# python-graphblas/python-graphblas

Hardware: AMD Instinct MI355X
Metric: GTEPS (mxv) on R-MAT scale-24 (higher is better)
Workload: dtype f32

## Files before the change

include/grb_mi355x.h:

```cpp
#ifndef GRB_MI355X_H
#define GRB_MI355X_H

#include <stdbool.h>
#include <stddef.h>
#include <stdint.h>

#ifdef __cplusplus
extern "C" {
#endif

#define GRB_VERSION 2
#define GRB_SUBVERSION 0

typedef uint64_t GrB_Index;
#define GrB_INDEX_MAX ((GrB_Index)(1ULL << 60) - 1)

typedef enum {
    GrB_SUCCESS = 0,
    GrB_NO_VALUE = 1,
    GrB_UNINITIALIZED_OBJECT = -1,
    GrB_NULL_POINTER = -2,
    GrB_INVALID_VALUE = -3,
    GrB_INVALID_INDEX = -4,
    GrB_DOMAIN_MISMATCH = -5,
// ... 133 lines not shown
    extern GrB_BinaryOp GrB_FIRST_##T, GrB_SECOND_##T, GrB_ONEB_##T, GxB_PAIR_##T, GrB_PLUS_##T, GrB_MINUS_##T,        \
        GrB_TIMES_##T, GrB_MIN_##T, GrB_MAX_##T, GxB_ANY_##T, GxB_LOR_##T, GxB_LAND_##T, GxB_LXOR_##T;                 \
      \
    extern GrB_BinaryOp GrB_EQ_##T, GrB_NE_##T, GrB_GT_##T, GrB_LT_##T, GrB_GE_##T, GrB_LE_##T;                        \
    extern GrB_Monoid GxB_ANY_##T##_MONOID;                                                                            \
    extern GrB_Semiring GxB_ANY_PAIR_##T, GxB_ANY_FIRST_##T, GxB_ANY_SECOND_##T;
GRB_FOR_EACH_TNAME(GRB_DECL_BINOPS)
#undef GRB_DECL_BINOPS
extern GrB_BinaryOp GrB_LOR, GrB_LAND, GrB_LXOR, GrB_LXNOR;
extern GrB_Monoid GrB_LOR_MONOID_BOOL, GrB_LAND_MONOID_BOOL, GrB_LXOR_MONOID_BOOL, GrB_LXNOR_MONOID_BOOL;

#define GRB_DECL_NUMERIC_OPS(T)                                                                                        \
    extern GrB_Monoid GrB_PLUS_MONOID_##T, GrB_TIMES_MONOID_##T, GrB_MIN_MONOID_##T, GrB_MAX_MONOID_##T;               \
    extern GrB_Semiring GrB_PLUS_TIMES_SEMIRING_##T, GrB_PLUS_MIN_SEMIRING_##T, GrB_MIN_PLUS_SEMIRING_##T,             \
        GrB_MIN_TIMES_SEMIRING_##T, GrB_MIN_FIRST_SEMIRING_##T, GrB_MIN_SECOND_SEMIRING_##T,                           \
        GrB_MIN_MAX_SEMIRING_##T, GrB_MAX_PLUS_SEMIRING_##T, GrB_MAX_TIMES_SEMIRING_##T,                               \
        GrB_MAX_FIRST_SEMIRING_##T, GrB_MAX_SECOND_SEMIRING_##T, GrB_MAX_MIN_SEMIRING_##T;                             \
    extern GrB_Semiring GxB_PLUS_PLUS_##T, GxB_PLUS_PAIR_##T, GxB_PLUS_FIRST_##T, GxB_PLUS_SECOND_##T,                 \
        GxB_PLUS_MAX_##T, GxB_MIN_MIN_##T, GxB_MAX_MAX_##T, GxB_MIN_PAIR_##T, GxB_MAX_PAIR_##T, GxB_TIMES_TIMES_##T,   \
        GxB_TIMES_PLUS_##T;
GRB_FOR_EACH_NUMERIC(GRB_DECL_NUMERIC_OPS)
#undef GRB_DECL_NUMERIC_OPS

extern GrB_Semiring GrB_LOR_LAND_SEMIRING_BOOL, GrB_LAND_LOR_SEMIRING_BOOL, GrB_LXOR_LAND_SEMIRING_BOOL,
    GrB_LXNOR_LOR_SEMIRING_BOOL;
extern GrB_Semiring GxB_LOR_LOR_BOOL, GxB_LAND_LAND_BOOL, GxB_LOR_FIRST_BOOL, GxB_LOR_SECOND_BOOL, GxB_LOR_PAIR_BOOL,
    GxB_LAND_FIRST_BOOL, GxB_LAND_SECOND_BOOL, GxB_LOR_LXOR_BOOL, GxB_LAND_LXOR_BOOL, GxB_LXOR_LOR_BOOL,
    GxB_LXOR_LXOR_BOOL, GxB_LXOR_FIRST_BOOL, GxB_LXOR_SECOND_BOOL, GxB_LXOR_PAIR_BOOL;

#define GRB_FOR_EACH_POSITIONAL(X) X(FIRSTI) X(FIRSTI1) X(FIRSTJ) X(FIRSTJ1) X(SECONDI) X(SECONDI1) X(SECONDJ) X(SECONDJ1)
#define GRB_DECL_POSITIONAL(P)                                                                                         \
    extern GrB_BinaryOp GxB_##P##_INT32, GxB_##P##_INT64;                                                              \
    extern GrB_Semiring GxB_MIN_##P##_INT32, GxB_MIN_##P##_INT64, GxB_MAX_##P##_INT32, GxB_MAX_##P##_INT64,            \
        GxB_ANY_##P##_INT32, GxB_ANY_##P##_INT64, GxB_PLUS_##P##_INT32, GxB_PLUS_##P##_INT64;
GRB_FOR_EACH_POSITIONAL(GRB_DECL_POSITIONAL)
#undef GRB_DECL_POSITIONAL


GrB_Info GrX_Matrix_import_CSR_device(GrB_Matrix *A, GrB_Type type, GrB_Index nrows, GrB_Index ncols,
                                      const int64_t *d_Ap, const int32_t *d_Aj, const void *d_Ax, GrB_Index nvals,
                                      int iso, int copy);
GrB_Info GxB_init(GrB_Mode mode, void *(*user_malloc)(size_t), void *(*user_calloc)(size_t, size_t),
                  void *(*user_realloc)(void *, size_t), void (*user_free)(void *));
GrB_Info GxB_Matrix_import_CSR(GrB_Matrix *A, GrB_Type type, GrB_Index nrows, GrB_Index ncols, GrB_Index **Ap, GrB_Index **Aj,
                               void **Ax, GrB_Index Ap_size, GrB_Index Aj_size, GrB_Index Ax_size, bool iso, bool jumbled,
                               const GrB_Descriptor desc);
GrB_Info GxB_Matrix_pack_CSR(GrB_Matrix A, GrB_Index **Ap, GrB_Index **Aj, void **Ax, GrB_Index Ap_size, GrB_Index Aj_size,
                             GrB_Index Ax_size, bool iso, bool jumbled, const GrB_Descriptor desc);
GrB_Info GrX_Matrix_hint_ranked(GrB_Matrix A, int ranked);
GrB_Info GrX_Matrix_shard_setup(GrB_Matrix A, const uint32_t *col_counts, int on_device, const GrB_Matrix like);
GrB_Info GrX_Matrix_export_CSR_device(const int64_t **d_Ap, const int32_t **d_Aj, const void **d_Ax, GrB_Index *nvals,
                                      int *iso, const GrB_Matrix A);
GrB_Info GrX_Vector_import_dense_device(GrB_Vector *v, GrB_Type type, GrB_Index n, const void *d_val,
                                        const uint32_t *d_present);
GrB_Info GrX_Vector_export_dense_device(const void **d_val, const uint32_t **d_present, const GrB_Vector v);
GrB_Info GrX_Vector_pin_natural(GrB_Vector v, int pinned);
GrB_Info GrX_Vector_modified(GrB_Vector v);
GrB_Info GrX_Matrix_cache_transpose(GrB_Matrix A);
GrB_Info GrX_get_stream(void **hip_stream);
GrB_Info GrX_set_stream(void *hip_stream);
GrB_Info GrX_synchronize(void);
GrB_Info GrX_trim_memory(void);
GrB_Info GrX_timer_start(void);
GrB_Info GrX_timer_stop(float *elapsed_ms);
typedef struct {
    int64_t kernel_launches;
    int64_t tiles;
    int64_t flops;
    int64_t out_nvals;
    int32_t method;
    int32_t fused_epilogue;
    int64_t hot_k;
    int64_t long_entries;
    int64_t long_segments;
    int32_t long_kernel;
    int32_t reorders;
    int64_t ordered;
    int64_t value_dict;
    int64_t fill_absent;
    int64_t long_probe;
    int64_t long_tails;
    int64_t pinned_natural;
    int64_t cold_tile_mode;
} GrX_Stats;
GrB_Info GrX_last_stats(GrX_Stats *stats);
GrB_Info GrX_mxm_streamed(const GrB_Semiring semiring, const GrB_Matrix A, const GrB_Matrix B, uint64_t budget_bytes,
                          uint64_t *nvals, uint64_t *checksum, uint64_t *flops, uint64_t *batches);
GrB_Info GrX_Matrix_isclose(bool *result, const GrB_Matrix A, const GrB_Matrix B, double rel_tol, double abs_tol);
GrB_Info GrX_Matrix_dup_as(GrB_Matrix *C, const GrB_Type type, const GrB_Matrix A);
GrB_Info GrX_Vector_dup_as(GrB_Vector *w, const GrB_Type type, const GrB_Vector u);
GrB_Info GrX_Vector_fill_absent(GrB_Vector v, const GrB_Monoid monoid);
GrB_Info GrX_Matrix_cache_bytes(const GrB_Matrix A, uint64_t *bytes);
GrB_Info GrX_option_set(const char *name, int64_t value);
GrB_Info GrX_option_get(const char *name, int64_t *value);
GrB_Info GrX_options_reset(void);
const char *GrX_version_string(void);

#define GRB_DECL_UNARY(T)                                                                                              \
    extern GrB_UnaryOp GrB_IDENTITY_##T, GrB_AINV_##T, GrB_MINV_##T, GrB_ABS_##T, GxB_ONE_##T, GxB_LNOT_##T;           \
    extern GrB_IndexUnaryOp GrB_VALUEEQ_##T, GrB_VALUENE_##T, GrB_VALUEGT_##T, GrB_VALUEGE_##T, GrB_VALUELT_##T,       \
        GrB_VALUELE_##T;                                                                                               \
    extern GrB_BinaryOp GrB_DIV_##T, GxB_RDIV_##T, GxB_RMINUS_##T, GxB_ISEQ_##T, GxB_ISNE_##T, GxB_ISGT_##T,           \
        GxB_ISLT_##T, GxB_ISGE_##T, GxB_ISLE_##T, GxB_POW_##T;
GRB_FOR_EACH_TNAME(GRB_DECL_UNARY)
#undef GRB_DECL_UNARY
extern GrB_UnaryOp GrB_LNOT, GrB_BNOT_INT8, GrB_BNOT_INT16, GrB_BNOT_INT32, GrB_BNOT_INT64, GrB_BNOT_UINT8, GrB_BNOT_UINT16,
    GrB_BNOT_UINT32, GrB_BNOT_UINT64;
extern GrB_IndexUnaryOp GrB_ROWINDEX_INT32, GrB_ROWINDEX_INT64, GrB_COLINDEX_INT32, GrB_COLINDEX_INT64, GrB_DIAGINDEX_INT32,
    GrB_DIAGINDEX_INT64, GrB_TRIL, GrB_TRIU, GrB_DIAG, GrB_OFFDIAG, GrB_COLLE, GrB_COLGT, GrB_ROWLE, GrB_ROWGT;

GrB_Info GrB_Scalar_new(GrB_Scalar *s, GrB_Type type);
GrB_Info GrB_Scalar_dup(GrB_Scalar *s, const GrB_Scalar t);
GrB_Info GrB_Scalar_free(GrB_Scalar *s);
GrB_Info GrB_Scalar_clear(GrB_Scalar s);
GrB_Info GrB_Scalar_nvals(GrB_Index *nvals, const GrB_Scalar s);
GrB_Info GrB_Scalar_wait(GrB_Scalar s, GrB_WaitMode mode);
GrB_Info GrB_Scalar_error(const char **error, const GrB_Scalar s);

GrB_Info GrB_Vector_apply(GrB_Vector w, const GrB_Vector mask, const GrB_BinaryOp accum, const GrB_UnaryOp op, const GrB_Vector u, const GrB_Descriptor desc);
GrB_Info GrB_Matrix_apply(GrB_Matrix C, const GrB_Matrix Mask, const GrB_BinaryOp accum, const GrB_UnaryOp op, const GrB_Matrix A, const GrB_Descriptor desc);
GrB_Info GrB_Vector_eWiseAdd_Semiring(GrB_Vector w, const GrB_Vector mask, const GrB_BinaryOp accum, const GrB_Semiring op, const GrB_Vector u, const GrB_Vector v, const GrB_Descriptor desc);
GrB_Info GrB_Vector_eWiseMult_Semiring(GrB_Vector w, const GrB_Vector mask, const GrB_BinaryOp accum, const GrB_Semiring op, const GrB_Vector u, const GrB_Vector v, const GrB_Descriptor desc);
#define GRB_DECL_MAT_BINARY(FN, HANDLE) \
    GrB_Info FN(GrB_Matrix C, const GrB_Matrix Mask, const GrB_BinaryOp accum, const HANDLE op, const GrB_Matrix A, const GrB_Matrix B, const GrB_Descriptor desc);
GRB_DECL_MAT_BINARY(GrB_Matrix_eWiseAdd_BinaryOp, GrB_BinaryOp)
GRB_DECL_MAT_BINARY(GrB_Matrix_eWiseAdd_Monoid, GrB_Monoid)
GRB_DECL_MAT_BINARY(GrB_Matrix_eWiseAdd_Semiring, GrB_Semiring)
GRB_DECL_MAT_BINARY(GrB_Matrix_eWiseMult_BinaryOp, GrB_BinaryOp)
GRB_DECL_MAT_BINARY(GrB_Matrix_eWiseMult_Monoid, GrB_Monoid)
GRB_DECL_MAT_BINARY(GrB_Matrix_eWiseMult_Semiring, GrB_Semiring)
GrB_Info GxB_Matrix_eWiseUnion(GrB_Matrix C, const GrB_Matrix Mask, const GrB_BinaryOp accum, const GrB_BinaryOp add, const GrB_Matrix A, const GrB_Scalar alpha, const GrB_Matrix B, const GrB_Scalar beta, const GrB_Descriptor desc);
GrB_Info GxB_Vector_eWiseUnion(GrB_Vector w, const GrB_Vector mask, const GrB_BinaryOp accum, const GrB_BinaryOp add, const GrB_Vector u, const GrB_Scalar alpha, const GrB_Vector v, const GrB_Scalar beta, const GrB_Descriptor desc);
GRB_DECL_MAT_BINARY(GrB_Matrix_kronecker_BinaryOp, GrB_BinaryOp)
GRB_DECL_MAT_BINARY(GrB_Matrix_kronecker_Monoid, GrB_Monoid)
GRB_DECL_MAT_BINARY(GrB_Matrix_kronecker_Semiring, GrB_Semiring)
#undef GRB_DECL_MAT_BINARY
GrB_Info GrB_Matrix_assign(GrB_Matrix C, const GrB_Matrix Mask, const GrB_BinaryOp accum, const GrB_Matrix A, const GrB_Index *I, GrB_Index ni, const GrB_Index *J, GrB_Index nj, const GrB_Descriptor desc);
GrB_Info GrB_Row_assign(GrB_Matrix C, const GrB_Vector mask, const GrB_BinaryOp accum, const GrB_Vector u, GrB_Index i, const GrB_Index *J, GrB_Index nj, const GrB_Descriptor desc);
GrB_Info GrB_Col_assign(GrB_Matrix C, const GrB_Vector mask, const GrB_BinaryOp accum, const GrB_Vector u, const GrB_Index *I, GrB_Index ni, GrB_Index j, const GrB_Descriptor desc);
GrB_Info GrB_Matrix_extract(GrB_Matrix C, const GrB_Matrix Mask, const GrB_BinaryOp accum, const GrB_Matrix A, const GrB_Index *I, GrB_Index ni, const GrB_Index *J, GrB_Index nj, const GrB_Descriptor desc);
GrB_Info GrB_Col_extract(GrB_Vector w, const GrB_Vector mask, const GrB_BinaryOp accum, const GrB_Matrix A, const GrB_Index *I, GrB_Index ni, GrB_Index j, const GrB_Descriptor desc);
GrB_Info GrB_Matrix_reduce_BinaryOp(GrB_Vector w, const GrB_Vector mask, const GrB_BinaryOp accum, const GrB_BinaryOp op, const GrB_Matrix A, const GrB_Descriptor desc);
GrB_Info GrB_Matrix_reduce_Monoid_Scalar(GrB_Scalar s, const GrB_BinaryOp accum, const GrB_Monoid monoid, const GrB_Matrix A, const GrB_Descriptor desc);
GrB_Info GrB_Vector_reduce_Monoid_Scalar(GrB_Scalar s, const GrB_BinaryOp accum, const GrB_Monoid monoid, const GrB_Vector u, const GrB_Descriptor desc);
GrB_Info GrB_Matrix_removeElement(GrB_Matrix C, GrB_Index i, GrB_Index j);
GrB_Info GrB_Matrix_diag(GrB_Matrix *C, const GrB_Vector v, int64_t k);
GrB_Info GxB_Vector_diag(GrB_Vector v, const GrB_Matrix A, int64_t k, const GrB_Descriptor desc);
GrB_Info GxB_Matrix_sort(GrB_Matrix C, GrB_Matrix P, GrB_BinaryOp op, const GrB_Matrix A, const GrB_Descriptor desc);
GrB_Info GxB_Vector_sort(GrB_Vector w, GrB_Vector p, GrB_BinaryOp op, const GrB_Vector u, const GrB_Descriptor desc);
GrB_Info GrX_sort_limits(int64_t *wave_max, int64_t *lds_max);
GrB_Info GrX_sort_last(int64_t rows_by_path[3]);
GrB_Info GrX_Matrix_reverse_rows(GrB_Matrix C, const GrB_Matrix A);
GrB_Info GrX_Vector_reverse(GrB_Vector w, const GrB_Vector u);
GrB_Info GrB_Vector_assign_Scalar(GrB_Vector w, const GrB_Vector mask, const GrB_BinaryOp accum, const GrB_Scalar s, const GrB_Index *I, GrB_Index ni, const GrB_Descriptor desc);
GrB_Info GrB_Vector_setElement_Scalar(GrB_Vector w, const GrB_Scalar s, GrB_Index i);
GrB_Info GrB_Vector_extractElement_Scalar(GrB_Scalar s, const GrB_Vector u, GrB_Index i);
GrB_Info GrB_Matrix_assign_Scalar(GrB_Matrix C, const GrB_Matrix Mask, const GrB_BinaryOp accum, const GrB_Scalar s, const GrB_Index *I, GrB_Index ni, const GrB_Index *J, GrB_Index nj, const GrB_Descriptor desc);
GrB_Info GrB_Matrix_setElement_Scalar(GrB_Matrix C, const GrB_Scalar s, GrB_Index i, GrB_Index j);
GrB_Info GrB_Matrix_extractElement_Scalar(GrB_Scalar s, const GrB_Matrix A, GrB_Index i, GrB_Index j);
GrB_Info GrB_Vector_select_Scalar(GrB_Vector w, const GrB_Vector mask, const GrB_BinaryOp accum, const GrB_IndexUnaryOp op, const GrB_Vector u, const GrB_Scalar y, const GrB_Descriptor desc);
GrB_Info GrB_Matrix_select_Scalar(GrB_Matrix C, const GrB_Matrix Mask, const GrB_BinaryOp accum, const GrB_IndexUnaryOp op, const GrB_Matrix A, const GrB_Scalar y, const GrB_Descriptor desc);
GrB_Info GrB_Vector_apply_BinaryOp1st_Scalar(GrB_Vector w, const GrB_Vector mask, const GrB_BinaryOp accum, const GrB_BinaryOp op, const GrB_Scalar x, const GrB_Vector u, const GrB_Descriptor desc);
GrB_Info GrB_Vector_apply_BinaryOp2nd_Scalar(GrB_Vector w, const GrB_Vector mask, const GrB_BinaryOp accum, const GrB_BinaryOp op, const GrB_Vector u, const GrB_Scalar y, const GrB_Descriptor desc);
GrB_Info GrB_Vector_apply_IndexOp_Scalar(GrB_Vector w, const GrB_Vector mask, const GrB_BinaryOp accum, const GrB_IndexUnaryOp op, const GrB_Vector u, const GrB_Scalar y, const GrB_Descriptor desc);
GrB_Info GrB_Matrix_apply_BinaryOp1st_Scalar(GrB_Matrix C, const GrB_Matrix Mask, const GrB_BinaryOp accum, const GrB_BinaryOp op, const GrB_Scalar x, const GrB_Matrix A, const GrB_Descriptor desc);
GrB_Info GrB_Matrix_apply_BinaryOp2nd_Scalar(GrB_Matrix C, const GrB_Matrix Mask, const GrB_BinaryOp accum, const GrB_BinaryOp op, const GrB_Matrix A, const GrB_Scalar y, const GrB_Descriptor desc);
// ... 30 lines not shown
```

python-graphblas_amd/_lib.py:

```python
from __future__ import annotations

import ctypes
import os

_HERE = os.path.dirname(os.path.abspath(__file__))
DEFAULT_LIB = os.path.join(_HERE, "csrc", "libgrb_mi355x.so")

lib = None
_handles = {}

c_void_p = ctypes.c_void_p
c_u64 = ctypes.c_uint64
c_int = ctypes.c_int

TYPE_NAMES = ["BOOL", "INT8", "INT16", "INT32", "INT64", "UINT8", "UINT16", "UINT32", "UINT64", "FP32", "FP64"]

GrB_SUCCESS = 0
GrB_NO_VALUE = 1


class GrX_Stats(ctypes.Structure):
    _fields_ = [("kernel_launches", ctypes.c_int64), ("tiles", ctypes.c_int64), ("flops", ctypes.c_int64),
                ("out_nvals", ctypes.c_int64), ("method", ctypes.c_int32), ("fused_epilogue", ctypes.c_int32),
                ("hot_k", ctypes.c_int64), ("long_entries", ctypes.c_int64), ("long_segments", ctypes.c_int64),
                ("long_kernel", ctypes.c_int32), ("reorders", ctypes.c_int32), ("ordered", ctypes.c_int64), ("value_dict", ctypes.c_int64), ("fill_absent", ctypes.c_int64),
                ("long_probe", ctypes.c_int64), ("long_tails", ctypes.c_int64), ("pinned_natural", ctypes.c_int64), ("cold_tile_mode", ctypes.c_int64)]


def load(path: str | None = None):
    global lib
    if lib is not None:
        return lib
    path = path or os.environ.get("GRB_MI355X_LIB") or DEFAULT_LIB
    if not os.path.exists(path):
        raise ImportError(
            f"{path} not found: build it with `python -c 'import __graft_entry__ as g; g.build()'` "
            "(there is no pure-Python or CPU fallback)"
        )
    if os.path.basename(path) == os.path.basename(DEFAULT_LIB):
        _share_hip_runtime_with_torch()
    lib = ctypes.CDLL(path)
    _declare(lib)
    return lib


def _share_hip_runtime_with_torch():
    import importlib.util
    import sys

    if "torch" in sys.modules:
        return
    try:
        spec = importlib.util.find_spec("torch")
    except (ImportError, ValueError):
        spec = None
    if spec is None or not spec.submodule_search_locations:
        return
    cand = os.path.join(list(spec.submodule_search_locations)[0], "lib", "libamdhip64.so")
    if os.path.exists(cand):
        try:
            ctypes.CDLL(cand, mode=ctypes.RTLD_GLOBAL)
        except OSError:
            pass


def _declare(L):
    P = ctypes.POINTER
    L.GrB_init.argtypes = [c_int]
    L.GrB_finalize.argtypes = []
    for name in ("GrB_mxm", "GrB_mxv", "GrB_vxm"):
        getattr(L, name).argtypes = [c_void_p] * 7
    L.GrB_Matrix_new.argtypes = [P(c_void_p), c_void_p, c_u64, c_u64]
    L.GrB_Matrix_dup.argtypes = [P(c_void_p), c_void_p]
    L.GrB_Matrix_free.argtypes = [P(c_void_p)]
    L.GrB_Matrix_clear.argtypes = [c_void_p]
    L.GrB_Matrix_resize.argtypes = [c_void_p, c_u64, c_u64]
    L.GrB_Matrix_reduce_Monoid.argtypes = [c_void_p] * 6
    for name in ("GrB_Matrix_nrows", "GrB_Matrix_ncols", "GrB_Matrix_nvals", "GrB_Vector_size", "GrB_Vector_nvals"):
        getattr(L, name).argtypes = [P(c_u64), c_void_p]
    L.GrB_Matrix_wait.argtypes = [c_void_p, c_int]
    L.GrB_Vector_wait.argtypes = [c_void_p, c_int]
    L.GrB_Matrix_error.argtypes = [P(ctypes.c_char_p), c_void_p]
    L.GrB_Vector_error.argtypes = [P(ctypes.c_char_p), c_void_p]
    L.GrB_Matrix_exportSize.argtypes = [P(c_u64), P(c_u64), P(c_u64), c_int, c_void_p]
    L.GxB_Matrix_import_CSR.argtypes = [P(c_void_p), c_void_p, c_u64, c_u64, P(c_void_p), P(c_void_p), P(c_void_p), c_u64, c_u64, c_u64,
                                        ctypes.c_bool, ctypes.c_bool, c_void_p]
    L.GxB_Matrix_pack_CSR.argtypes = [c_void_p, P(c_void_p), P(c_void_p), P(c_void_p), c_u64, c_u64, c_u64, ctypes.c_bool, ctypes.c_bool, c_void_p]
    L.GrB_transpose.argtypes = [c_void_p] * 5
    L.GrB_Vector_new.argtypes = [P(c_void_p), c_void_p, c_u64]
    L.GrB_Vector_dup.argtypes = [P(c_void_p), c_void_p]
    L.GrB_Vector_free.argtypes = [P(c_void_p)]
    L.GrB_Vector_clear.argtypes = [c_void_p]
    L.GrB_Vector_removeElement.argtypes = [c_void_p, c_u64]
    for kind in ("Vector", "Matrix"):
        for call in ("eWiseAdd", "eWiseMult"):
            for opclass in ("BinaryOp", "Monoid", "Semiring"):
                getattr(L, f"GrB_{kind}_{call}_{opclass}").argtypes = [c_void_p] * 7
    for kind in ("Vector", "Matrix"):
        getattr(L, f"GxB_{kind}_eWiseUnion").argtypes = [c_void_p] * 9
    L.GrB_Matrix_diag.argtypes = [P(c_void_p), c_void_p, ctypes.c_int64]
    L.GxB_Vector_diag.argtypes = [c_void_p, c_void_p, ctypes.c_int64, c_void_p]
    L.GxB_Matrix_sort.argtypes = [c_void_p] * 5
    L.GxB_Vector_sort.argtypes = [c_void_p] * 5
    L.GrX_sort_limits.argtypes = [P(ctypes.c_int64), P(ctypes.c_int64)]
    L.GrX_sort_last.argtypes = [P(ctypes.c_int64)]
    L.GrX_Matrix_reverse_rows.argtypes = [c_void_p, c_void_p]
    L.GrX_Vector_reverse.argtypes = [c_void_p, c_void_p]
    for opclass in ("BinaryOp", "Monoid", "Semiring"):
        getattr(L, f"GrB_Matrix_kronecker_{opclass}").argtypes = [c_void_p] * 7
# ... 93 lines not shown
```

python-graphblas_amd/csrc/grb_context.hip:

```cpp
#include <chrono>
#include <algorithm>
#include <cctype>
#include <cstdlib>
#include <cstring>
#include <mutex>
#include <unordered_map>
#include <vector>

#include "grb_internal.hpp"

namespace grb {

#ifdef GRB_ABLATE
static constexpr int DEBUG_FLAGS_MASK = ~0;
#else
static constexpr int DEBUG_FLAGS_MASK = 128 | 256 | 2048 | 65536;
#endif


Context &ctx()
{
    static Context c;
    return c;
}
// ... 115 lines not shown
            c.host_stage = nullptr;
            c.host_stage_failed = true;
        }
        return c.host_stage;
    }
    return nullptr;
}
void preload_stage() { (void)stage_block(4096); (void)stage_block(STAGE_BYTES); }
static bool trace_copies()
{
    static const bool on = [] { const char *e = getenv("GRB_TRACE_COPIES"); return e && atoi(e) != 0; }();
    return on;
}
struct CopyTrace {
    const char *what;
    size_t bytes;
    bool staged;
    std::chrono::steady_clock::time_point t0;
    CopyTrace(const char *w, size_t b, bool s) : what(w), bytes(b), staged(s), t0(std::chrono::steady_clock::now()) {}
    ~CopyTrace()
    {
        if (!trace_copies()) return;
        const double ms = std::chrono::duration<double, std::milli>(std::chrono::steady_clock::now() - t0).count();
        if (ms > 0.5) fprintf(stderr, "[grb copy] %s %zu bytes %s: %.2f ms\n", what, bytes, staged ? "staged" : "direct", ms);
    }
};
void h2d(void *dst, const void *src, size_t bytes)
{
    if (!bytes) return;
    Context &c = ctx();
    if (void *st = stage_block(bytes)) {
        CopyTrace tr("h2d", bytes, true);
        memcpy(st, src, bytes);
        GRB_HIP(hipMemcpyAsync(dst, st, bytes, hipMemcpyHostToDevice, c.stream));
        GRB_HIP(hipStreamSynchronize(c.stream));
        return;
    }
    CopyTrace tr("h2d", bytes, false);
    GRB_HIP(hipMemcpyAsync(dst, src, bytes, hipMemcpyHostToDevice, c.stream));
    GRB_HIP(hipStreamSynchronize(c.stream));
}
void d2h(void *dst, const void *src, size_t bytes)
{
    Context &c = ctx();
    if (bytes) {
        if (void *st = stage_block(bytes)) {
            CopyTrace tr("d2h", bytes, true);
            GRB_HIP(hipMemcpyAsync(st, src, bytes, hipMemcpyDeviceToHost, c.stream));
            GRB_HIP(hipStreamSynchronize(c.stream));
            memcpy(dst, st, bytes);
            return;
        }
        CopyTrace tr("d2h", bytes, false);
        GRB_HIP(hipMemcpyAsync(dst, src, bytes, hipMemcpyDeviceToHost, c.stream));
        GRB_HIP(hipStreamSynchronize(c.stream));
        return;
    }
    GRB_HIP(hipStreamSynchronize(c.stream));
}
void d2d(void *dst, const void *src, size_t bytes)
{
    if (bytes) GRB_HIP(hipMemcpyAsync(dst, src, bytes, hipMemcpyDeviceToDevice, ctx().stream));
}
void sync_stream() { GRB_HIP(hipStreamSynchronize(ctx().stream)); }

namespace {
struct Option {
    const char *name;
    int Context::*i;
    int64_t Context::*l;
    enum Rule { ANY, WITHIN, ONE_OF, CLAMP } rule;
    int64_t lo, hi;
    bool (*hook)(int64_t &value);
};
using Hook = bool (*)(int64_t &);
constexpr int64_t MAX64 = INT64_MAX, P30 = 1 << 30;
constexpr Option opt(const char *n, int Context::*f, Option::Rule r = Option::ANY, int64_t lo = 0, int64_t hi = 0, Hook h = nullptr) { return {n, f, nullptr, r, lo, hi, h}; }
constexpr Option opt(const char *n, int64_t Context::*f, Option::Rule r = Option::ANY, int64_t lo = 0, int64_t hi = 0, Hook h = nullptr) { return {n, nullptr, f, r, lo, hi, h}; }

bool known_debug_flags(int64_t &v) { return !((int)v & ~DEBUG_FLAGS_MASK); }
bool short_kernel_exists(int64_t &v) { return v != 2 && v != 3 && v != 4; }
bool snap_long_classes(int64_t &v) { if (v != 16 && v != 32 && v != 64) v = 8; return true; }
bool window_group(int64_t &v) { return (v & (v - 1)) == 0; }
bool explicit_cold_layout(int64_t &) { ctx().ctile_code = 0; return true; }
bool release_cache_when_off(int64_t &v) { if (!v) dev_cache_release(); return true; }

const Option OPTIONS[] = {
    opt("debug_flags", &Context::debug_flags, Option::ANY, 0, 0, known_debug_flags),
    opt("pull_ipt", &Context::tune_pull_ipt),
    opt("hot_min_cols", &Context::hot_min_cols),
    opt("hot_k", &Context::hot_k),
    opt("push_mode", &Context::push_mode),
    opt("split_min_nnz", &Context::split_min_nnz),
    opt("split_min_len", &Context::split_min_len, Option::CLAMP, 0, P30),
    opt("short_kernel", &Context::short_kernel, Option::WITHIN, 0, 6, short_kernel_exists),
    opt("lazy_layout", &Context::lazy_layout),
    opt("lazy_min_nnz", &Context::lazy_min_nnz),
    opt("lean_min_nnz", &Context::lean_min_nnz, Option::CLAMP, 0, MAX64),
    opt("long_kernel", &Context::long_kernel),
    opt("long_classes", &Context::long_classes, Option::ANY, 0, 0, snap_long_classes),
    opt("long_sub", &Context::long_sub, Option::CLAMP, 0, 16),
    opt("long_sub_min_len", &Context::long_sub_min_len),
    opt("mxm_mask_mode", &Context::mxm_mask_mode),
    opt("mat_write_kernel", &Context::mat_write_kernel, Option::WITHIN, 0, 1),
    opt("mxm_heavy_kernel", &Context::mxm_heavy_kernel),
    opt("drop_hot_cols", &Context::drop_hot_cols),
    opt("mxm_unit_min_flops", &Context::mxm_unit_min_flops),
    opt("mxm_unit_min_per_window", &Context::mxm_unit_min_per_window),
    opt("mxm_masked_units_min_flops", &Context::mxm_masked_units_min_flops),
    opt("mxm_unit_small", &Context::mxm_unit_small, Option::WITHIN, 1, P30),
    opt("mxm_unit_mid", &Context::mxm_unit_mid, Option::WITHIN, 1, P30),
    opt("mxm_unit_dense", &Context::mxm_unit_dense, Option::WITHIN, 1, P30),
    opt("mxm_sym_windows", &Context::mxm_sym_windows, Option::WITHIN, 1, 64),
    opt("mxm_window_groups", &Context::mxm_window_groups, Option::WITHIN, 0, 8, window_group),
    opt("mxm_xcd_map", &Context::mxm_xcd_map, Option::WITHIN, 0, 1),
    opt("mxm_checksum_pass", &Context::mxm_checksum_pass, Option::WITHIN, 0, 1),
    opt("mxm_bitmap_pool_mb", &Context::mxm_bitmap_pool_mb),
    opt("mxm_bitmap_min_cnt", &Context::mxm_bitmap_min_cnt),
    opt("mxm_bitmap_pool_cap", &Context::mxm_bitmap_pool_cap),
    opt("vec_pad_min_bytes", &Context::vec_pad_min_bytes),
    opt("hub_min_len", &Context::hub_min_len, Option::CLAMP, 0, P30),
    opt("fill_absent", &Context::fill_absent, Option::WITHIN, 0, 1),
    opt("rows_tile", &Context::rows_tile, Option::WITHIN, 0, 2),
    opt("lazy_tagged", &Context::lazy_tagged, Option::WITHIN, 0, 1),
    opt("ctile_pack", &Context::ctile_pack, Option::WITHIN, 0, 2, explicit_cold_layout),
    opt("ctile_code", &Context::ctile_code, Option::WITHIN, 0, 1),
    opt("strip_slot16", &Context::strip_slot16, Option::WITHIN, 0, 1),
    opt("rtile_pack", &Context::rtile_pack, Option::WITHIN, 0, 1),
    opt("cold_in_rows", &Context::cold_in_rows, Option::CLAMP, 0, P30),
    opt("stream_nt_min_nnz", &Context::stream_nt_min_nnz, Option::CLAMP, 0, MAX64),
    opt("bool_probe", &Context::bool_probe, Option::WITHIN, 0, 16),
    opt("rtile_rows", &Context::rtile_rows, Option::ONE_OF, 8192, 16384),
    opt("rtile_entries", &Context::rtile_entries, Option::WITHIN, 256, 1 << 24),
    opt("rows_head", &Context::rows_head, Option::WITHIN, 0, 1),
    opt("rows_head_min_groups", &Context::rows_head_min_groups, Option::CLAMP, 0, MAX64),
    opt("push_small", &Context::push_small, Option::WITHIN, 0, 1),
    opt("value_dict", &Context::value_dict, Option::WITHIN, 0, 1),
    opt("order_mode", &Context::order_mode, Option::WITHIN, 0, 1),
    opt("order_min_nnz", &Context::order_min_nnz, Option::CLAMP, 0, MAX64),
    opt("alloc_cache", &Context::alloc_cache, Option::ANY, 0, 0, release_cache_when_off),
};
constexpr size_t N_OPTIONS = sizeof(OPTIONS) / sizeof(OPTIONS[0]);
int64_t option_initial[N_OPTIONS];

const Option *option_find(const char *name)
{
    for (const Option &o : OPTIONS)
        if (!strcmp(o.name, name)) return &o;
    return nullptr;
}
int64_t option_load(const Option &o) { return o.i ? (int64_t)(ctx().*o.i) : ctx().*o.l; }
GrB_Info option_store(const Option &o, int64_t v)
{
    if (o.rule == Option::WITHIN && (v < o.lo || v > o.hi)) return GrB_INVALID_VALUE;
    if (o.rule == Option::ONE_OF && v != o.lo && v != o.hi) return GrB_INVALID_VALUE;
    if (o.rule == Option::CLAMP) v = std::max(o.lo, std::min(v, o.hi));
    if (o.hook && !o.hook(v)) return GrB_INVALID_VALUE;
    if (o.i) ctx().*o.i = (int)v;
    else ctx().*o.l = v;
    return GrB_SUCCESS;
}
}

}

using namespace grb;

extern "C" GrB_Info GrB_init(GrB_Mode mode)
{
    Context &c = ctx();
    if (c.initialized) return GrB_INVALID_VALUE;
    if (mode != GrB_BLOCKING && mode != GrB_NONBLOCKING) return GrB_INVALID_VALUE;
    int ndev = 0;
    if (hipGetDeviceCount(&ndev) != hipSuccess || ndev <= 0) {
        (void)hipGetLastError();
        return GrB_PANIC;
    }
    int dev = 0;
    if (hipGetDevice(&dev) != hipSuccess) return GrB_PANIC;
    c.device = dev;
    {
        int cus = 0;
        if (hipDeviceGetAttribute(&cus, hipDeviceAttributeMultiprocessorCount, dev) == hipSuccess && cus > 0) c.num_cus = cus;
    }
    c.blocking = (mode == GrB_BLOCKING);
    c.stream = nullptr;
    hipMemPool_t pool;
    if (hipDeviceGetDefaultMemPool(&pool, dev) == hipSuccess) {
        uint64_t thresh = UINT64_MAX;
        (void)hipMemPoolSetAttribute(pool, hipMemPoolAttrReleaseThreshold, &thresh);
    }
    (void)hipGetLastError();
    if (hipEventCreate(&c.ev0) != hipSuccess || hipEventCreate(&c.ev1) != hipSuccess) return GrB_PANIC;
    if (const char *e = getenv("GRB_PRELOAD"); !e || atoi(e) != 0) {
        preload_mxv();
        preload_mxm();
        preload_vecops();
        preload_object();
        preload_prim();
        preload_select();
        preload_extract();
        preload_apply();
        preload_assign();
        preload_kron();
        preload_diag();
        preload_mxv_posn();
        preload_sort();
        preload_stage();
    }
// ... 146 lines not shown
```

python-graphblas_amd/csrc/grb_internal.hpp:

```cpp
#pragma once
#include <hip/hip_runtime.h>

#include <cstdint>
#include <cstdio>
#include <cstring>
#include <memory>
#include <string>
#include <type_traits>

#include "grb_mi355x.h"

namespace grb {

enum TypeCode : int {
    TC_BOOL = 0, TC_INT8, TC_INT16, TC_INT32, TC_INT64, TC_UINT8, TC_UINT16, TC_UINT32, TC_UINT64, TC_FP32, TC_FP64,
    TC_COUNT
};

enum OpCode : int {
    OP_NONE = -1,
    OP_FIRST = 0, OP_SECOND, OP_PAIR, OP_PLUS, OP_MINUS, OP_RMINUS, OP_TIMES, OP_MIN, OP_MAX,
    OP_LOR, OP_LAND, OP_LXOR, OP_LXNOR, OP_ANY, OP_COUNT,
    OP_EQ = 32, OP_NE, OP_GT, OP_LT, OP_GE, OP_LE,
    OP_UNSUPPORTED = 1000
// ... 20 lines not shown
constexpr uint64_t MAGIC_VECTOR = 0x4752425645435452ULL;
constexpr uint64_t MAGIC_MATRIX = 0x4752424d41545258ULL;
constexpr uint64_t MAGIC_FREED = 0xdeadbeefdeadbeefULL;

struct Error {
    GrB_Info info;
    std::string msg;
};

[[noreturn]] inline void fail(GrB_Info info, const std::string &msg) { throw Error{info, msg}; }

#define GRB_HIP(expr)                                                                                       \
    do {                                                                                                    \
        hipError_t _e = (expr);                                                                             \
        if (_e != hipSuccess) {                                                                             \
            ::grb::fail(_e == hipErrorOutOfMemory ? GrB_OUT_OF_MEMORY : GrB_PANIC,                          \
                        std::string("HIP error '") + hipGetErrorString(_e) + "' at " __FILE__ ":" +        \
                            std::to_string(__LINE__) + " in " #expr);                                       \
        }                                                                                                   \
    } while (0)

struct Context {
    bool initialized = false;
    bool blocking = false;
    int device = 0;
    int num_cus = 256;
    hipStream_t stream = nullptr;
    void (*host_free)(void *) = nullptr;
    hipEvent_t ev0 = nullptr, ev1 = nullptr;
    int64_t vec_pad_min_bytes = 1 << 20;
    int alloc_cache = 1;
    int drop_hot_cols = 1;
    int mxm_heavy_kernel = 1;
    int mxm_unit_small = 512, mxm_unit_mid = 1024, mxm_unit_dense = 4096;
    int64_t mxm_unit_min_flops = 1024;
    int64_t mxm_unit_min_per_window = 16;
    int64_t mxm_masked_units_min_flops = 64ll << 20;
    int64_t mxm_bitmap_pool_cap = INT32_MAX;
    int64_t mxm_window_groups = 0;
    int mxm_xcd_map = 1;
    int mxm_checksum_pass = 0;
    int64_t mxm_sym_windows = 8;
    int mxm_bitmap_min_cnt = 512;
    int64_t mxm_bitmap_pool_mb = 16384;
    int mat_write_kernel = 1;
    int mxm_mask_mode = 1;
    int long_sub = 0;
    int long_sub_min_len = 0;
    int long_kernel = 5;
    int short_kernel = 6;
    int64_t lean_min_nnz = 48ll << 20;
    GrX_Stats stats{};
    int debug_flags = 0;
    int tune_pull_ipt = 0;
    int64_t hot_min_cols = 1 << 20;
    int64_t hot_k = 0;
    int64_t split_min_nnz = 1 << 22;
    int split_min_len = 0;
    int long_classes = 16;
    int lazy_layout = 1;
    int64_t lazy_min_nnz = 1 << 22;
    int push_mode = 1;
    int rows_tile = 1;
    int64_t stream_nt_min_nnz = 48ll << 20;
    int bool_probe = 8;
    int rtile_rows = 8192;
    int64_t rtile_entries = 49152;
    int rows_head = 1;
    int64_t rows_head_min_groups = 16384;
    int push_small = 1;
    int fill_absent = 1;
    int hub_min_len = 1024;
    int value_dict = 1;
    int order_mode = 1;
    int64_t order_min_nnz = 24ll << 20;
    int64_t reorder_count = 0;
    void *host_stage = nullptr;
    bool host_stage_failed = false;
    void *host_pinned = nullptr;
    unsigned long long *push_counters = nullptr;
    int push_parity = 0;
    int lazy_tagged = 1;
    int ctile_code = 1;
    int ctile_pack = 0;
    int strip_slot16 = 1;
    int rtile_pack = 1;
    int cold_in_rows = 0;
};
Context &ctx();
void require_init();

void *dev_alloc(size_t bytes);
void *dev_alloc_zero(size_t bytes);
void dev_free(void *p);
void dev_cache_release();
void h2d(void *dst, const void *src, size_t bytes);
void d2h(void *dst, const void *src, size_t bytes);
void d2d(void *dst, const void *src, size_t bytes);
void sync_stream();

template <typename T>
struct DevBuf {
    T *p = nullptr;
    explicit DevBuf(size_t n, bool zero = false)
    {
        p = static_cast<T *>(zero ? dev_alloc_zero(sizeof(T) * (n ? n : 1)) : dev_alloc(sizeof(T) * (n ? n : 1)));
    }
    DevBuf(const DevBuf &) = delete;
    DevBuf &operator=(const DevBuf &) = delete;
    ~DevBuf() { dev_free(p); }
    T *release()
    {
        T *q = p;
        p = nullptr;
        return q;
    }
};

void preload_mxv();
void preload_stage();
void preload_mxm();
void preload_vecops();
void preload_object();
void preload_prim();
void preload_select();
void preload_extract();
void preload_apply();
void preload_assign();
void preload_kron();
void preload_diag();
void preload_mxv_posn();
void preload_sort();

template <typename T>
struct DevPtr {
    T *p = nullptr;
    DevPtr() = default;
    explicit DevPtr(T *q) : p(q) {}
    DevPtr(const DevPtr &) = delete;
    DevPtr &operator=(const DevPtr &) = delete;
    DevPtr(DevPtr &&o) noexcept : p(o.release()) {}
    DevPtr &operator=(DevPtr &&o) noexcept
    {
        if (this != &o) reset(o.release());
        return *this;
    }
    ~DevPtr() { dev_free(p); }
    void reset(T *q = nullptr)
    {
        dev_free(p);
        p = q;
    }
    T *get() const { return p; }
    operator T *() const { return p; }
    T *release()
    {
        T *q = p;
        p = nullptr;
        return q;
    }
};

inline int64_t ceil_div(int64_t a, int64_t b) { return (a + b - 1) / b; }
inline size_t bits_words64(uint64_t n) { return (size_t)((n + 63) / 64); }
inline dim3 grid1d(int64_t threads)
{
// ... 42 lines not shown
    bool builtin;
};

struct GB_Perm {
    int64_t refs = 1;
    uint64_t n = 0;
    int32_t *d_rank = nullptr;
    int32_t *d_inv = nullptr;
    int64_t n_live_rows = 0;
    int64_t n_live_cols = 0;
};

constexpr size_t VEC_VAL_PAD = (size_t)8 << 20;
constexpr size_t VEC_BITS_PAD = (size_t)256 << 10;

struct GB_Vector_opaque {
    uint64_t magic;
    GrB_Type type;
    uint64_t n;
    void *d_val;
    uint64_t *d_bits;
    bool padded;
    int64_t nvals;
    GB_Perm *order = nullptr;
    bool exported = false;
    bool pinned = false;
    std::string err;
};

struct GB_Matrix_opaque;
namespace grb {
void matrix_free(GB_Matrix_opaque *A);
struct MatrixDeleter {
    void operator()(GB_Matrix_opaque *A) const { matrix_free(A); }
};
using MatrixOwner = std::unique_ptr<GB_Matrix_opaque, MatrixDeleter>;
}

struct GB_Matrix_opaque {
    struct TileTable {
        grb::DevPtr<int64_t> d_tile_row;
        int64_t n_tiles = 0;
        int tile_items = 0;
        uint64_t bytes() const { return d_tile_row ? 8ull * (uint64_t)(n_tiles + 1) : 0; }
    };
    struct HotCols {
        grb::DevPtr<int32_t> d_col_hot;
        grb::DevPtr<int32_t> d_hot_cols;
        int64_t hot_k = 0;
        int hot_state = 0;
        bool hot_cols_dropped = false;
        uint64_t bytes() const { return d_hot_cols ? 4ull * (uint64_t)hot_k : 0; }
    };
    struct ValueDict {
        grb::DevPtr<void> d_vdict;
        int vdict_n = 0;
        double vals_absmax = 0.0;
        bool vals_finite = false;
        grb::DevPtr<unsigned long long> d_vd_table;
        grb::DevPtr<unsigned char> d_vd_codes;
    };
    struct Strips {
        grb::DevPtr<unsigned long long> d_sstart;
        grb::DevPtr<int32_t> d_sslot;
        grb::DevPtr<uint16_t> d_sslot16;
        grb::DevPtr<int32_t> d_sslot_base;
        int64_t strip_cb[161] = {0};
        int strip_ncls = 8;
        int hub_ncls = 0;
        int hub_lds_lim = 0;
        grb::DevPtr<int32_t> d_wg_tab;
        grb::DevPtr<int64_t> d_strip_cb;
        int wg_tab_g = 0;
        int64_t strip_nseg = 0;
        grb::DevPtr<char> d_hrec;
        int hrec_bytes = 0;
        uint64_t hot_bytes() const;
    };
    struct ColdTiles {
        grb::DevPtr<int32_t> d_ct_col;
        grb::DevPtr<void> d_ct_val;
        grb::DevPtr<uint16_t> d_ct_loc;
        grb::DevPtr<void> d_ct_tiles;
        grb::DevPtr<int32_t> d_ct_order;
        int64_t ct_xoff[9] = {0};
        int64_t ct_ntiles = 0;
        int64_t ct_units = 0;
        int ct_mode = 0;
        uint64_t bytes(uint64_t vs) const;
    };
    struct TaggedGroups {
        grb::DevPtr<int32_t> d_tg_off;
        grb::DevPtr<int32_t> d_tg_col;
        grb::DevPtr<void> d_tg_val;
        grb::DevPtr<unsigned char> d_tg_tag;
        grb::DevPtr<uint64_t> d_tg_nonempty;
        int64_t tg_units = 0;
        int tg_state = 0;
        uint64_t bytes(uint64_t nrows, uint64_t vs, bool dict) const;
    };
    struct RowTiles {
        grb::DevPtr<int32_t> d_rt_col;
        grb::DevPtr<uint16_t> d_rt_tag;
        grb::DevPtr<void> d_rt_val;
        grb::DevPtr<void> d_rt_tiles;
        grb::DevPtr<int32_t> d_rt_order;
        grb::DevPtr<unsigned int> d_rt_counter;
        int64_t rt_units = 0;
        int rt_ntiles = 0;
        int rt_rows4 = 0;
        int rt_state = 0;
        uint64_t bytes(uint64_t vs, bool dict) const;
    };
    struct RowSplit {
        int split_state = 0;
        bool split_hot = false;
        int split_kind = 0;
        bool short_tagged_only = false;
        int64_t tails_max_len = 0;
        grb::MatrixOwner short_part;
        int64_t n_long = 0, n_chunks = 0;
        grb::DevPtr<uint64_t> d_long_bits;
        grb::DevPtr<int32_t> d_long_rows;
        grb::DevPtr<int32_t> d_chunk_slot;
        grb::DevPtr<int64_t> d_chunk_start;
        grb::DevPtr<int32_t> d_chunk_len;
        grb::DevPtr<int32_t> d_long_prefix;
        grb::DevPtr<int32_t> d_probe;
        int probe_k = 0;
        grb::DevPtr<int32_t> d_lcol;
        grb::DevPtr<void> d_lval;
        int64_t long_nnz = 0;
        int cls_lds_lim = 0;
        grb::DevPtr<int64_t> d_it_start;
        grb::DevPtr<int32_t> d_it_len;
        grb::DevPtr<int32_t> d_it_slot;
        grb::DevPtr<int64_t> d_item_begin;
        int64_t item_begin[9] = {0};
        int64_t n_items = 0;
        Strips strips;
        ColdTiles cold;
        TaggedGroups tagged;
        RowTiles rtile;
        uint64_t bytes(uint64_t nrows, uint64_t vs, bool dict) const;
    };
    struct VertexOrder {
        GB_Perm *perm = nullptr;
        bool col_order_only = false;
        GB_Matrix_opaque *ord = nullptr;
        int ord_state = 0;
        uint64_t ord_sig = 0;
        int64_t ord_live_rows = 0;
        grb::DevPtr<int32_t> d_cold_bounds;
        int ct_ncr = 0;
    };

    uint64_t magic;
    GrB_Type type;
    uint64_t nrows, ncols;
    int64_t nvals = 0;
    int64_t *d_ptr = nullptr;
    int32_t *d_col = nullptr;
    void *d_val = nullptr;
    bool iso = false;
    bool owns = true;
    GB_Matrix_opaque *tr = nullptr;
// ... 126 lines not shown
```

python-graphblas_amd/csrc/grb_mxv.hip:

```cpp
#include <algorithm>
#include <cstring>
#include <vector>

#include "grb_internal.hpp"
#include "grb_ops.hpp"

namespace grb {

#include "grb_mxv_common.inc"
#include "grb_mxv_pull.inc"
#include "grb_mxv_long.inc"
#include "grb_mxv_vdict.inc"
#include "grb_mxv_strip.inc"
#include "grb_mxv_rows.inc"
#include "grb_mxv_rows_tag.inc"
#include "grb_mxv_ctile.inc"
#include "grb_mxv_rtile.inc"
#include "grb_mxv_split_build.inc"
#include "grb_mxv_write.inc"
#include "grb_mxv_push.inc"
#include "grb_mxv_hot.inc"
#include "grb_mxv_order.inc"

static int64_t hot_table_size(int64_t n, size_t value_bytes)
// ... 210 lines not shown
        sp.d_chunk_slot.reset((int32_t *)dev_alloc(sizeof(int32_t) * (size_t)nc));
        sp.d_chunk_start.reset((int64_t *)dev_alloc(sizeof(int64_t) * (size_t)nc));
        sp.d_chunk_len.reset((int32_t *)dev_alloc(sizeof(int32_t) * (size_t)nc));
        sp.d_long_prefix.reset((int32_t *)dev_alloc(sizeof(int32_t) * (size_t)bits_words64((uint64_t)m)));
        GRB_DISPATCH_TYPE(A->type->code, T, {
            hipLaunchKernelGGL((k_split_fill<T>), dim3((unsigned)ceil_div(m, 256)), dim3(256), 0, ctx().stream,
                               (const int64_t *)A->d_ptr, col_src, (const T *)A->d_val, A->iso ? 1 : 0, m, min_len,
                               (const int64_t *)S->d_ptr, (const int64_t *)lflag.p, (const int64_t *)nchunk.p, S->d_col,
                               (T *)S->d_val, sp.d_long_rows, sp.d_chunk_slot, sp.d_chunk_start, sp.d_chunk_len, sp.d_long_prefix);
            if (tail_max > 0)
                hipLaunchKernelGGL((k_split_fill_tails<T>), dim3((unsigned)ceil_div(nl, 4)), dim3(256), 0, ctx().stream, (const int64_t *)A->d_ptr, col_src,
                                   (const T *)A->d_val, A->iso ? 1 : 0, (const int32_t *)sp.d_long_rows, nl, (const int64_t *)S->d_ptr, S->d_col, (T *)S->d_val,
                                   tail_max, tail_lim);
        })
        if (A->type->code == TC_BOOL && kind == 1 && nl * 16 < 0x7fffffffll) {
            sp.d_probe.reset((int32_t *)dev_alloc(sizeof(int32_t) * (size_t)(nl * 16)));
            hipLaunchKernelGGL(k_probe_fill, dim3((unsigned)ceil_div(nl * 16, 256)), dim3(256), 0, ctx().stream, (const int64_t *)A->d_ptr, col_src,
                               (const int32_t *)sp.d_long_rows, nl, 16, sp.d_probe);
            sp.probe_k = 16;
        }
        const int64_t nnz_long = nnz - nnz_short;
        DevBuf<int64_t> lpre(tail_max > 0 ? nl + 1 : 0);
        int64_t nnz_keyed = nnz_long;
        if (tail_max > 0) {
            hipLaunchKernelGGL(k_long_lens, dim3((unsigned)ceil_div(nl + 1, 256)), dim3(256), 0, ctx().stream, (const int64_t *)A->d_ptr, (const int32_t *)sp.d_long_rows, nl, lpre.p);
            prim_exclusive_sum_i64(lpre.p, lpre.p, nl + 1);
            d2h(&nnz_keyed, lpre.p + nl, 8);
        }
        if (nnz_keyed < 0xf0000000ll && nnz < 0xffffffffll) {
            const bool strips = kind == 2 || kind == 4;
            const int ncls = (strips && (ctx().long_classes == 16 || ctx().long_classes == 32 || ctx().long_classes == 64))
                                 ? ctx().long_classes : 8;
            const int COLD_CLS = 8;
            const int64_t lds_lim4 = std::min<int64_t>(hot ? A->hot.hot_k : 0, long_lds_codes((int)A->type->size, A->type->code == TC_BOOL, LONG_LDS_WORDS) / 8 * ncls);
            const int64_t codes_total = (int64_t)A->ncols + ((hot && !A->hot_identity) ? A->hot.hot_k : 0);
            const int range_cls = kind == 4 ? COLD_CLS : ncls;
            unsigned sub = 1;
            if (ctx().long_sub > 0) sub = (unsigned)std::min(kind == 4 ? 8 : 16, ctx().long_sub);
            else if (A->type->code != TC_BOOL || kind == 4) {
                const int64_t image_bytes = A->type->code == TC_BOOL ? (int64_t)A->ncols / 8 : (int64_t)A->ncols * (int64_t)A->type->size;
                while (sub < (kind == 4 ? 8u : 16u) && image_bytes > (int64_t)sub * range_cls * (3ll << 20)) sub *= 2;
            }
            const int64_t sub_min_len = kind == 4 ? 0 : (ctx().long_sub_min_len > 0 ? ctx().long_sub_min_len : 512 * (int64_t)sub);
            const int64_t nv = (int64_t)ncls * (int64_t)sub * nl;
            int bits = 1;
            while (((int64_t)1 << bits) < nv) bits++;
            DevBuf<uint64_t> keys(nnz_keyed), keys2(nnz_keyed);
            DevBuf<uint32_t> idx(nnz_keyed), idx2(nnz_keyed);
            const bool own_ranges = kind == 4 && A->hot_identity && A->order.d_cold_bounds && A->order.ct_ncr > 0;
            const int hub_ncls = (own_ranges && ctx().hub_min_len > 0 && ncls < 64) ? 64 : 0;
            const int64_t hub_lim = hub_ncls ? std::min<int64_t>((int64_t)A->ncols, long_lds_codes((int)A->type->size, A->type->code == TC_BOOL, LONG_LDS_WORDS) / 8 * hub_ncls) : 0;
            const int64_t hub_len = hub_ncls ? (int64_t)ctx().hub_min_len : 0;
            if (tail_max > 0 && (!own_ranges || (int64_t)tail_lim != lds_lim4 || (hub_ncls && tail_max > hub_len)))
                fail(GrB_PANIC, "long / short split: the cold entries of the long rows were cut at another limit than the class keys use (internal error)");
            const unsigned discard_cls = (unsigned)(ncls + hub_ncls + (own_ranges ? A->order.ct_ncr : COLD_CLS * (int)sub));
            if (kind == 4)
                hipLaunchKernelGGL(k_long_keys, dim3((unsigned)nl), dim3(256), 0, ctx().stream, (const int64_t *)A->d_ptr,
                                   (const int64_t *)S->d_ptr, (const int32_t *)sp.d_long_rows, col_src, nl, keys.p, idx.p,
                                   (unsigned)lds_lim4, (unsigned)std::max<int64_t>(1, ceil_div(codes_total - std::max<int64_t>(lds_lim4, hot ? A->hot.hot_k : 0), (int64_t)COLD_CLS * (int64_t)sub)),
                                   sub, sub_min_len, (unsigned)ncls, 2, (unsigned)(hot ? A->hot.hot_k : 0),
                                   own_ranges ? (const int32_t *)A->order.d_cold_bounds : (const int32_t *)nullptr, own_ranges ? A->order.ct_ncr + 1 : 0,
                                   hub_len, (unsigned)hub_lim, (unsigned)hub_ncls, tail_max, discard_cls, tail_max > 0 ? (const int64_t *)lpre.p : (const int64_t *)nullptr);
            else
            hipLaunchKernelGGL(k_long_keys, dim3((unsigned)nl), dim3(256), 0, ctx().stream, (const int64_t *)A->d_ptr,
                               (const int64_t *)S->d_ptr, (const int32_t *)sp.d_long_rows, col_src, nl, keys.p, idx.p,
                               (unsigned)(hot ? A->hot.hot_k : 0), (unsigned)std::max<int64_t>(1, ceil_div((int64_t)A->ncols, (int64_t)ncls * (int64_t)sub)),
                               sub, sub_min_len, (unsigned)ncls, kind == 2 ? 1 : 0, 0u, (const int32_t *)nullptr, 0, (int64_t)0, 0u, 0u, (int64_t)0, 0u, (const int64_t *)nullptr);
            const int nvc = ncls + hub_ncls;
            const int n_cr = own_ranges ? A->order.ct_ncr : COLD_CLS * (int)sub;
            const int nvirt = kind == 4 ? nvc + n_cr + (tail_max > 0 ? 1 : 0) : ncls * (int)sub;
            const int hot_cls = 0;
            const unsigned strip_sub = kind == 4 ? 1u : sub;
            if (strips) {
                int vbits = 1;
                while ((1 << vbits) < nvirt) vbits++;
                prim_sort_pairs_u64_u32_bits(keys.p, keys2.p, idx.p, idx2.p, nnz_keyed, 32, 32 + vbits);
            } else {
                prim_sort_pairs_u64_u32(keys.p, keys2.p, idx.p, idx2.p, nnz_keyed, bits);
            }
            int ct_mode = 0;
            std::vector<int32_t> h_bounds;
            if (kind == 4 && ctx().ctile_code == 1 && ctx().ctile_pack == 0 && A->vd.vdict_n > 0 && A->type->size == 4 && A->type->code != TC_BOOL && !A->iso && codes_total <= ((int64_t)1 << 24))
                ct_mode = 3;
            if (kind == 4 && own_ranges && ctx().ctile_pack > 0) {
                h_bounds.resize((size_t)A->order.ct_ncr + 1);
                d2h(h_bounds.data(), A->order.d_cold_bounds, sizeof(int32_t) * h_bounds.size());
                int64_t widest = 0;
                for (int r = 0; r < A->order.ct_ncr; r++) widest = std::max<int64_t>(widest, (int64_t)h_bounds[(size_t)r + 1] - (int64_t)h_bounds[(size_t)r]);
                if (widest < ((int64_t)1 << 19) - 1) ct_mode = (ctx().ctile_pack == 2 && A->vd.vdict_n > 0 && A->type->size == 4 && !A->iso) ? 2 : 1;
            }
            const bool ct_packed = ct_mode == 1 || ct_mode == 2;
            const int ct_slots = ct_packed ? CT_PACK_SLOTS : (A->type->size > 4 ? CT_SLOTS / 2 : CT_SLOTS);
            const int n_sb = (int)ceil_div(nl, (int64_t)ct_slots);
            const int64_t n_tiles = kind == 4 ? (int64_t)n_cr * n_sb : 0;
            std::vector<int64_t> h_first((size_t)n_tiles + 1, 0);
            DevBuf<int64_t> tile_first(n_tiles + 1);
            int64_t n_strip = nnz_long;
            if (kind == 4) {
                hipLaunchKernelGGL(k_ctile_first, dim3((unsigned)ceil_div(n_tiles + 1, 256)), dim3(256), 0, ctx().stream, (const uint64_t *)keys2.p, nnz_keyed,
                                   n_tiles, n_sb, (unsigned)nvc, tile_first.p, ct_slots);
                d2h(h_first.data(), tile_first.p, sizeof(int64_t) * (size_t)(n_tiles + 1));
                n_strip = h_first[0];
                if (h_first[(size_t)n_tiles] != nnz_long)
                    fail(GrB_PANIC, "long / short split: the short part and the class keys disagree about the cold entries that moved (internal error)");
            }
            if (kind == 4) {
                sp.long_nnz = nnz_long;
                sp.strips.strip_ncls = ncls;
                sp.strips.hub_ncls = hub_ncls;
                sp.strips.hub_lds_lim = (int)hub_lim;
                sp.cls_lds_lim = (int)lds_lim4;
                for (int c = 0; c <= nvc; c++) sp.strips.strip_cb[c] = 0;
            }
            if (strips && n_strip > 0) {
                const int64_t nblk = ceil_div(n_strip, STRIP_CH);
                DevBuf<int64_t> blk(nblk + 1);
                hipLaunchKernelGGL(k_strip_count, dim3((unsigned)nblk), dim3(STRIP_CH), 0, ctx().stream, (const uint64_t *)keys2.p, n_strip, blk.p);
                prim_exclusive_sum_i64(blk.p, blk.p, nblk + 1);
                int64_t nseg = 0;
                d2h(&nseg, blk.p + nblk, 8);
                if (nseg >= 0x7ffffff0ll) fail(GrB_NOT_IMPLEMENTED, "class strips: too many segments for 32-bit numbering");
                DevBuf<int64_t> seg_first(nseg + 1), off(nseg + 1);
                hipLaunchKernelGGL(k_strip_seg_fill, dim3((unsigned)nblk), dim3(STRIP_CH), 0, ctx().stream, (const uint64_t *)keys2.p, n_strip,
                                   (const int64_t *)blk.p, seg_first.p);
                hipLaunchKernelGGL(k_strip_plen, dim3((unsigned)ceil_div(nseg + 1, 256)), dim3(256), 0, ctx().stream, (const int64_t *)seg_first.p,
                                   nseg, off.p);
                prim_exclusive_sum_i64(off.p, off.p, nseg + 1);
                constexpr int MAXC = 160;
                DevBuf<int64_t> sc(MAXC + 1), raw(MAXC + 1), cshift(MAXC);
                hipLaunchKernelGGL(k_strip_class_bounds, dim3(1), dim3(128), 0, ctx().stream, (const uint64_t *)keys2.p, (const int64_t *)seg_first.p,
                                   nseg, nl, strip_sub, (const int64_t *)off.p, sc.p, raw.p, nvc, hot_cls);
                int64_t h_raw[MAXC + 1], h_shift[MAXC], h_cb[MAXC + 1];
                d2h(h_raw, raw.p, sizeof(int64_t) * (size_t)(nvc + 1));
                int64_t base = 0;
                for (int c = 0; c < nvc; c++) {
                    h_cb[c] = base / STRIP_CH;
                    h_shift[c] = base - h_raw[c];
                    base += ceil_div(h_raw[c + 1] - h_raw[c], STRIP_CH) * STRIP_CH;
                }
                h_cb[nvc] = base / STRIP_CH;
                const int64_t padded = base, nch = padded / STRIP_CH;
                h2d(cshift.p, h_shift, sizeof(int64_t) * (size_t)nvc);
                sp.cls_lds_lim = (int)lds_lim4;
                const int64_t hot_chunks = kind == 4 ? h_cb[nvc] : 0;
                const int64_t flat_entries = kind == 4 ? 0 : padded;
                const int code_bytes = A->type->code == TC_BOOL ? 32 : 16;
                const bool use_dict = A->vd.vdict_n > 0;
                const int val_bytes = A->iso ? 0 : (use_dict ? 8 : (int)std::max<size_t>(16, 8 * A->type->size));
                if (padded > 0 && padded < 0x7fffffff0ll) {
                    sp.d_lcol.reset((int32_t *)dev_alloc(sizeof(int32_t) * (size_t)std::max<int64_t>(flat_entries, 1)));
                    sp.d_lval.reset(A->iso ? nullptr : dev_alloc(A->type->size * (size_t)std::max<int64_t>(flat_entries, 1)));
                    sp.strips.d_sstart.reset((unsigned long long *)dev_alloc(sizeof(unsigned long long) * (size_t)nch));
                    sp.strips.d_sslot.reset((int32_t *)dev_alloc(sizeof(int32_t) * (size_t)(padded / 8)));
                    GRB_HIP(hipMemsetAsync(sp.strips.d_sslot, 0xff, sizeof(int32_t) * (size_t)(padded / 8), ctx().stream));
                    GRB_HIP(hipMemsetAsync(sp.d_lcol, 0xff, sizeof(int32_t) * (size_t)std::max<int64_t>(flat_entries, 1), ctx().stream));
                    if (sp.d_lval) GRB_HIP(hipMemsetAsync(sp.d_lval, 0, A->type->size * (size_t)std::max<int64_t>(flat_entries, 1), ctx().stream));
                    GRB_HIP(hipMemsetAsync(sp.strips.d_sstart, 0, sizeof(unsigned long long) * (size_t)nch, ctx().stream));
                    if (kind == 4) {
                        sp.strips.hrec_bytes = code_bytes + val_bytes;
                        const size_t hbytes = (size_t)std::max<int64_t>(hot_chunks, 1) * 64 * (size_t)sp.strips.hrec_bytes;
                        sp.strips.d_hrec.reset((char *)dev_alloc(hbytes));
                        if (A->type->code == TC_BOOL) GRB_HIP(hipMemsetAsync(sp.strips.d_hrec, 0xff, hbytes, ctx().stream));
                        else {
                            const int64_t n_rec = std::max<int64_t>(hot_chunks, 1) * 64;
                            GRB_DISPATCH_TYPE(A->type->code, T, {
                                hipLaunchKernelGGL((k_hrec_init<T>), dim3((unsigned)ceil_div(n_rec, 256)), dim3(256), 0, ctx().stream, sp.strips.d_hrec, n_rec,
// ... 10 lines not shown
                                           use_dict ? (const unsigned long long *)A->vd.d_vd_table : (const unsigned long long *)nullptr,
                                           use_dict ? (const unsigned char *)A->vd.d_vd_codes : (const unsigned char *)nullptr, hub_ncls, (int)hub_lim);
                    })
                    {
                        int64_t h_end[MAXC];
                        for (int c = 0; c < nvc; c++) h_end[c] = h_cb[c + 1] * STRIP_CH;
                        DevBuf<int64_t> cend(MAXC);
                        h2d(cend.p, h_end, sizeof(int64_t) * (size_t)nvc);
                        hipLaunchKernelGGL(k_strip_pad_starts, dim3(1), dim3(128), 0, ctx().stream, (const int64_t *)sc.p, (const int64_t *)off.p,
                                           (const int64_t *)cshift.p, (const int64_t *)cend.p, nvc, sp.strips.d_sstart);
                        sync_stream();
                    }
                    if (ctx().strip_slot16 && nch > 0) {
                        DevBuf<unsigned int> too_wide(1, true);
                        DevPtr<uint16_t> s16((uint16_t *)dev_alloc(sizeof(uint16_t) * (size_t)(padded / 8)));
                        DevPtr<int32_t> sb((int32_t *)dev_alloc(sizeof(int32_t) * (size_t)nch));
                        hipLaunchKernelGGL(k_strip_slot16, dim3((unsigned)ceil_div(nch, 4)), dim3(256), 0, ctx().stream, (const int32_t *)sp.strips.d_sslot, nch, s16.get(), sb.get(), too_wide.p);
                        unsigned int wide = 0;
                        d2h(&wide, too_wide.p, sizeof(wide));
                        if (!wide) {
                            sp.strips.d_sslot16 = std::move(s16);
                            sp.strips.d_sslot_base = std::move(sb);
                            sp.strips.d_sslot.reset();
                        }
                    }
                    for (int c = 0; c <= nvc; c++) sp.strips.strip_cb[c] = h_cb[c];
                    if (hub_ncls > 0) {
                        const int G = std::max(nvc, ctx().num_cus);
                        std::vector<int> wgs((size_t)nvc, 0);
                        int used = 0;
                        for (int c = 0; c < nvc; c++)
                            if (h_cb[c + 1] > h_cb[c]) { wgs[(size_t)c] = 1; used++; }
                        while (used < G) {
                            int best = -1;
                            double best_load = -1.0;
                            for (int c = 0; c < nvc; c++) {
                                if (!wgs[(size_t)c]) continue;
                                const double load = (double)(h_cb[c + 1] - h_cb[c]) / wgs[(size_t)c];
                                if (load > best_load) { best_load = load; best = c; }
                            }
                            if (best < 0) break;
                            wgs[(size_t)best]++;
                            used++;
                        }
                        std::vector<int32_t> tab((size_t)G * 5, 0);
                        int b = 0;
                        std::vector<int> next((size_t)nvc, 0);
                        for (int round = 0; b < G; round++) {
                            bool any = false;
                            for (int c = 0; c < nvc && b < G; c++) {
                                if (next[(size_t)c] >= wgs[(size_t)c]) continue;
                                any = true;
                                int32_t *t = &tab[(size_t)b * 5];
                                t[0] = c;
                                t[1] = c < ncls ? c : c - ncls;
                                t[2] = c < ncls ? ncls : hub_ncls;
                                t[3] = next[(size_t)c]++;
                                t[4] = wgs[(size_t)c];
                                b++;
                            }
                            if (!any) break;
                        }
                        for (; b < G; b++) {
                            int32_t *t = &tab[(size_t)b * 5];
                            t[0] = 0; t[1] = 0; t[2] = ncls; t[3] = 1 << 28; t[4] = 1;
                        }
                        sp.strips.d_wg_tab.reset((int32_t *)dev_alloc(sizeof(int32_t) * tab.size()));
                        h2d(sp.strips.d_wg_tab, tab.data(), sizeof(int32_t) * tab.size());
                        sp.strips.d_strip_cb.reset((int64_t *)dev_alloc(sizeof(int64_t) * (size_t)(nvc + 1)));
                        h2d(sp.strips.d_strip_cb, h_cb, sizeof(int64_t) * (size_t)(nvc + 1));
                        sp.strips.wg_tab_g = G;
                    }
                    if (getenv("GRB_PRINT_STRIPS")) {
                        fprintf(stderr, "[strips kind %d] %d classes (%d of them the hub level's), chunks per class:", kind, nvc, hub_ncls);
                        for (int c = 0; c < nvc; c++) fprintf(stderr, " %lld", (long long)(h_cb[c + 1] - h_cb[c]));
                        fprintf(stderr, "  segments %lld\n", (long long)nseg);
                    }
                    sp.strips.strip_ncls = ncls;
                    sp.strips.strip_nseg = nseg;
                    sp.long_nnz = nnz_long;
                    sync_stream();
                }
            }
            const bool use_dict_all = ct_mode == 2 || ct_mode == 3;
            if (kind == 4 && nnz_long > n_strip) {
                std::vector<CTile> h_tiles;
                std::vector<int64_t> h_efirst;
                std::vector<int> tile_range;
                std::vector<int64_t> range_cnt((size_t)n_cr, 0);
                int64_t units = 0;
                for (int64_t t = 0; t < n_tiles; t++) {
                    const int64_t cnt = h_first[t + 1] - h_first[t];
                    if (cnt == 0) continue;
                    const int64_t pieces = ceil_div(cnt, CT_MAX_ENTRIES), per = ceil_div(cnt, pieces);
                    for (int64_t q = 0; q < pieces; q++) {
                        const int64_t e0 = h_first[t] + q * per, e1 = std::min<int64_t>(h_first[t] + (q + 1) * per, h_first[t + 1]);
                        CTile ct;
                        ct.u0 = units;
                        ct.n_units = (int32_t)ceil_div(e1 - e0, (int64_t)CT_EPL);
                        ct.base = (int32_t)((t % n_sb) * (int64_t)ct_slots);
                        units += ct.n_units;
                        h_tiles.push_back(ct);
                        h_efirst.push_back(e0);
                        tile_range.push_back((int)(t / n_sb));
                    }
                    range_cnt[(size_t)(t / n_sb)] += cnt;
                }
                const int64_t nt = (int64_t)h_tiles.size();
                h_efirst.push_back(nnz_long);
                std::vector<int> range_xcd((size_t)n_cr);
                if (own_ranges) {
                    std::vector<int> by_cnt((size_t)n_cr);
                    for (int r = 0; r < n_cr; r++) by_cnt[(size_t)r] = r;
                    std::stable_sort(by_cnt.begin(), by_cnt.end(), [&](int x, int y) { return range_cnt[(size_t)x] > range_cnt[(size_t)y]; });
                    int64_t load[8] = {0};
                    for (int r : by_cnt) {
                        int best = 0;
                        for (int x = 1; x < 8; x++)
                            if (load[x] < load[best]) best = x;
                        range_xcd[(size_t)r] = best;
                        load[best] += range_cnt[(size_t)r];
                    }
                } else {
                    for (int r = 0; r < n_cr; r++) range_xcd[(size_t)r] = r % 8;
                }
                std::vector<int32_t> h_order;
                h_order.reserve((size_t)nt);
                for (int x = 0; x < 8; x++) {
                    sp.cold.ct_xoff[x] = (int64_t)h_order.size();
                    for (int64_t t = 0; t < nt; t++)
                        if (range_xcd[(size_t)tile_range[(size_t)t]] == x) h_order.push_back((int32_t)t);
                }
                sp.cold.ct_xoff[8] = (int64_t)h_order.size();
                const size_t ents = (size_t)std::max<int64_t>(units, 1) * CT_EPL;
                sp.cold.d_ct_tiles.reset(dev_alloc((sizeof(CTile) + sizeof(int32_t)) * (size_t)std::max<int64_t>(nt, 1)));
                h2d(sp.cold.d_ct_tiles, h_tiles.data(), sizeof(CTile) * (size_t)nt);
                if (ct_packed) {
                    std::vector<int32_t> h_cbase((size_t)nt);
                    for (int64_t t = 0; t < nt; t++) h_cbase[(size_t)t] = h_bounds[(size_t)tile_range[(size_t)t]];
                    h2d((char *)sp.cold.d_ct_tiles.get() + sizeof(CTile) * (size_t)std::max<int64_t>(nt, 1), h_cbase.data(), sizeof(int32_t) * (size_t)nt);
                }
                sp.cold.d_ct_order.reset((int32_t *)dev_alloc(sizeof(int32_t) * (size_t)std::max<int64_t>(nt, 1)));
                h2d(sp.cold.d_ct_order, h_order.data(), sizeof(int32_t) * (size_t)nt);
                DevBuf<int64_t> efirst(nt + 1);
                h2d(efirst.p, h_efirst.data(), sizeof(int64_t) * (size_t)(nt + 1));
                sp.cold.d_ct_col.reset((int32_t *)dev_alloc(sizeof(int32_t) * ents));
                const size_t ct_vb = use_dict_all ? 1 : A->type->size;
                sp.cold.d_ct_val.reset((A->iso || ct_mode == 3) ? nullptr : dev_alloc(ct_vb * ents));
                sp.cold.d_ct_loc.reset(ct_packed ? nullptr : (uint16_t *)dev_alloc(sizeof(uint16_t) * ents));
                GRB_HIP(hipMemsetAsync(sp.cold.d_ct_col, 0xff, sizeof(int32_t) * ents, ctx().stream));
                if (sp.cold.d_ct_val) GRB_HIP(hipMemsetAsync(sp.cold.d_ct_val, 0, ct_vb * ents, ctx().stream));
                if (sp.cold.d_ct_loc) GRB_HIP(hipMemsetAsync(sp.cold.d_ct_loc, 0, sizeof(uint16_t) * ents, ctx().stream));
                if (ct_mode == 3 && nt > 0)
                    hipLaunchKernelGGL(k_ctile_pad_slots, dim3((unsigned)ceil_div(nt, 256)), dim3(256), 0, ctx().stream, (const CTile *)sp.cold.d_ct_tiles.get(),
                                       (const int64_t *)efirst.p, nt, sp.cold.d_ct_loc.get(), (uint16_t)ct_slots);
                const int64_t n_cold = nnz_long - n_strip;
                {
                    DevBuf<uint64_t> key2(n_cold), key2s(n_cold);
                    DevBuf<uint32_t> pay(n_cold), pays(n_cold);
                    hipLaunchKernelGGL(k_ctile_keys2, dim3((unsigned)ceil_div(n_cold, 256)), dim3(256), 0, ctx().stream, (const uint32_t *)idx2.p, n_strip, n_cold,
                                       (const int64_t *)efirst.p, nt, col_src, key2.p, pay.p);
                    int tbits = 1;
                    while (((int64_t)1 << tbits) < nt) tbits++;
                    prim_sort_pairs_u64_u32(key2.p, key2s.p, pay.p, pays.p, n_cold, 32 + tbits);
                    GRB_DISPATCH_TYPE(A->type->code, T, {
                        hipLaunchKernelGGL((k_ctile_place<T>), dim3((unsigned)ceil_div(n_cold, 256)), dim3(256), 0, ctx().stream, (const uint64_t *)keys2.p,
                                           (const uint32_t *)idx2.p, n_strip, n_cold, (const uint64_t *)key2s.p, (const uint32_t *)pays.p, (const int64_t *)efirst.p,
                                           (const CTile *)sp.cold.d_ct_tiles.get(), (const T *)A->d_val, A->iso ? 1 : 0, sp.cold.d_ct_col, (T *)sp.cold.d_ct_val.get(), sp.cold.d_ct_loc,
                                           use_dict_all ? (const unsigned long long *)A->vd.d_vd_table : (const unsigned long long *)nullptr,
                                           use_dict_all ? (const unsigned char *)A->vd.d_vd_codes : (const unsigned char *)nullptr,
                                           ct_packed ? (const int32_t *)((const char *)sp.cold.d_ct_tiles.get() + sizeof(CTile) * (size_t)std::max<int64_t>(nt, 1)) : (const int32_t *)nullptr,
                                           ct_mode == 3 ? 1 : 0);
                    })
                    sync_stream();
                }
                sp.cold.ct_mode = ct_mode;
                sp.cold.ct_ntiles = nt;
                sp.cold.ct_units = units;
                if (getenv("GRB_PRINT_STRIPS")) {
                    fprintf(stderr, "[cold tiles] mode %d (slots %d), %d column ranges, %lld tiles, entries per range:", ct_mode, ct_slots, n_cr, (long long)nt);
                    for (int r = 0; r < n_cr; r++) fprintf(stderr, " %lld(x%d)", (long long)range_cnt[(size_t)r], range_xcd[(size_t)r]);
                    fprintf(stderr, "\n");
                }
                sync_stream();
            }
            DevBuf<int64_t> vptr(strips ? 0 : nv + 1), icnt(strips ? 0 : nv + 1);
            if (!strips) {
            hipLaunchKernelGGL(k_long_vptr, dim3((unsigned)ceil_div(nv + 1, 256)), dim3(256), 0, ctx().stream,
                               (const uint64_t *)keys2.p, nnz_long, nv, vptr.p);
            hipLaunchKernelGGL(k_long_item_count, dim3((unsigned)ceil_div(nv + 1, 256)), dim3(256), 0, ctx().stream,
                               (const int64_t *)vptr.p, nv, icnt.p);
            prim_exclusive_sum_i64(icnt.p, icnt.p, nv + 1);
            int64_t ni = 0;
            d2h(&ni, icnt.p + nv, 8);
            if (ni > 0 && ni < 0x7fffffffll) {
                DevBuf<uint64_t> ikey(ni), ikey2(ni);
                DevBuf<uint32_t> iid(ni), iorder(ni);
                DevBuf<int64_t> isrc(ni), osrc(ni), len4(ni + 1);
                DevBuf<int32_t> ilen(ni), islot(ni);
                hipLaunchKernelGGL(k_long_item_fill, dim3((unsigned)ceil_div(nv, 256)), dim3(256), 0, ctx().stream,
                                   (const int64_t *)vptr.p, nv, nl, (const int64_t *)icnt.p, ikey.p, iid.p, isrc.p, ilen.p, islot.p);
                prim_sort_pairs_u64_u32(ikey.p, ikey2.p, iid.p, iorder.p, ni, 19);
                sp.d_it_len.reset((int32_t *)dev_alloc(sizeof(int32_t) * (size_t)ni));
                sp.d_it_slot.reset((int32_t *)dev_alloc(sizeof(int32_t) * (size_t)ni));
                sp.d_it_start.reset((int64_t *)dev_alloc(sizeof(int64_t) * (size_t)(ni + 1)));
                hipLaunchKernelGGL(k_long_item_order, dim3((unsigned)ceil_div(ni + 1, 256)), dim3(256), 0, ctx().stream,
                                   (const uint32_t *)iorder.p, ni, (const int64_t *)isrc.p, (const int32_t *)ilen.p,
                                   (const int32_t *)islot.p, osrc.p, sp.d_it_len, sp.d_it_slot, len4.p);
                prim_exclusive_sum_i64(len4.p, sp.d_it_start, ni + 1);
                int64_t padded = 0;
                d2h(&padded, sp.d_it_start + ni, 8);
                sp.d_item_begin.reset((int64_t *)dev_alloc(sizeof(int64_t) * 9));
                hipLaunchKernelGGL(k_long_class_bounds, dim3(1), dim3(64), 0, ctx().stream, (const uint64_t *)ikey2.p, ni, sp.d_item_begin, sub);
                d2h(sp.item_begin, sp.d_item_begin, sizeof(int64_t) * 9);
                sp.cls_lds_lim = (int)std::min<int64_t>(hot ? A->hot.hot_k : 0,
                                                        long_lds_codes((int)A->type->size, A->type->code == TC_BOOL, LONG_LDS_WORDS));
                sp.d_lcol.reset((int32_t *)dev_alloc(sizeof(int32_t) * (size_t)(padded + 2048)));
                sp.d_lval.reset(A->iso ? nullptr : dev_alloc(A->type->size * (size_t)(padded + 2048)));
                GRB_DISPATCH_TYPE(A->type->code, T, {
                    hipLaunchKernelGGL((k_long_place<T>), dim3((unsigned)ni), dim3(64), 0, ctx().stream, (const int64_t *)sp.d_it_start,
                                       (const int64_t *)osrc.p, (const int32_t *)sp.d_it_len, (const uint32_t *)idx2.p, col_src,
                                       (const T *)A->d_val, A->iso ? 1 : 0, sp.d_lcol, (T *)sp.d_lval.get(), sp.cls_lds_lim);
                })
                GRB_HIP(hipMemsetAsync(sp.d_lcol + padded, 0xff, sizeof(int32_t) * 2048, ctx().stream));
                if (sp.d_lval) GRB_HIP(hipMemsetAsync((char *)sp.d_lval.get() + A->type->size * (size_t)padded, 0, A->type->size * 2048, ctx().stream));
                sp.n_items = ni;
                sp.long_nnz = nnz_long;
                sync_stream();
            }
            }
        }
        sync_stream();
    }
    sp.d_long_bits.reset(lbits.release());
    sp.n_long = nl;
    sp.n_chunks = nc;
    sp.split_hot = hot;
    sp.split_kind = kind;
    sp.split_state = 1;
    sp.tails_max_len = tail_max;
    A->split = std::move(sp);
    if (want_tagged_only && S->nrows == A->nrows && S->nvals < 0x1ffffffffll) {
        ensure_tagged_index(A);
        if (ctx().rows_tile && (A->hot_identity || (hot && ctx().rows_tile == 2))) ensure_rtile(A);
        if (A->split.rtile.rt_state != 1 || !ctx().lazy_tagged) ensure_tagged(A);
        dev_free(S->d_col);
        S->d_col = nullptr;
        if (!S->iso) {
            dev_free(S->d_val);
            S->d_val = nullptr;
        }
        A->split.short_tagged_only = true;
    }
    if (hot && ctx().drop_hot_cols && nc > 0 && A->split.long_nnz > 0 && (kind == 1 || kind == 2 || kind == 4) && A->col_hot()) {
        if (A->hot_identity) {
            dev_free(A->d_col);
            A->d_col = nullptr;
        } else {
            A->hot.d_col_hot.reset();
        }
        A->hot.hot_cols_dropped = true;
    }
}

static uint64_t order_signature()
{
    const Context &c = ctx();
    uint64_t h = 1469598103934665603ull;
    const int64_t v[] = {c.long_kernel, c.short_kernel, c.long_classes, c.split_min_len, c.long_sub, c.long_sub_min_len, c.lean_min_nnz,
                         c.split_min_nnz, c.hot_k, c.drop_hot_cols, c.hub_min_len, c.value_dict, c.rows_tile, c.rtile_rows, c.rtile_entries, c.cold_in_rows, c.rtile_pack, c.strip_slot16, c.ctile_pack, c.ctile_code, c.lazy_tagged};
    for (int64_t x : v) h = (h ^ (uint64_t)x) * 1099511628211ull;
    return h;
}

static GB_Perm *ensure_perm(GB_Matrix_opaque *S, int64_t k_hot, DevBuf<unsigned int> &poscnt)
{
    const int64_t n = (int64_t)S->ncols, nnz = S->nvals;
    GB_Matrix_opaque *partner = S->tr ? S->tr : S->tr_of;
    const bool adopt = !S->order.perm && partner && partner->order.perm;
    if (adopt) {
        S->order.perm = partner->order.perm;
        perm_retain(S->order.perm);
    }
    DevBuf<unsigned int> cnt(n, true);
    const int hstride = nnz >= ((int64_t)1 << 26) ? 8 : 1;
    hipLaunchKernelGGL(k_hot_hist, dim3((unsigned)ceil_div(nnz, 256 * hstride)), dim3(256), 0, ctx().stream, S->d_col, nnz, cnt.p, hstride);
    if (S->order.perm) {
        hipLaunchKernelGGL(k_order_poscnt, dim3((unsigned)ceil_div(n, 256)), dim3(256), 0, ctx().stream, (const unsigned int *)cnt.p,
                           (const int32_t *)S->order.perm->d_inv, n, poscnt.p);
        sync_stream();
        return S->order.perm;
    }
    DevBuf<uint64_t> keys(n), keys2(n);
    DevBuf<uint32_t> ids(n), ids2(n);
    hipLaunchKernelGGL(k_order_keys, dim3((unsigned)ceil_div(n, 256)), dim3(256), 0, ctx().stream, (const unsigned int *)cnt.p, matrix_rowptr(S), n, keys.p, ids.p);
    prim_sort_pairs_u64_u32(keys.p, keys2.p, ids.p, ids2.p, n, 40);
    GB_Perm *P = new GB_Perm();
    P->n = (uint64_t)n;
    try {
        P->d_rank = (int32_t *)dev_alloc(sizeof(int32_t) * (size_t)n);
        P->d_inv = (int32_t *)dev_alloc(sizeof(int32_t) * (size_t)n);
        DevBuf<unsigned long long> live(2, true);
        hipLaunchKernelGGL(k_order_place, dim3((unsigned)ceil_div(n, 1024)), dim3(1024), 0, ctx().stream, (const uint32_t *)ids2.p, (const uint64_t *)keys2.p, n, k_hot,
                           P->d_rank, P->d_inv, poscnt.p, live.p);
        unsigned long long h_live[2] = {0, 0};
        d2h(h_live, live.p, sizeof(h_live));
        P->n_live_rows = (int64_t)h_live[0];
        P->n_live_cols = (int64_t)h_live[1];
    } catch (...) {
        perm_release(P);
        throw;
    }
    S->order.perm = P;
    if (partner && !partner->order.perm) {
        partner->order.perm = P;
        perm_retain(P);
    }
    return P;
}

static void ensure_ordered(GB_Matrix_opaque *S)
{
    const uint64_t sig = order_signature();
    if (S->order.ord_state == 1 && S->order.ord && S->order.ord_sig == sig) return;
    if (S->order.ord_state == -1 && S->order.ord_sig == sig) return;
    if (S->order.ord) {
        matrix_free(S->order.ord);
        S->order.ord = nullptr;
    }
    S->order.ord_state = -1;
    S->order.ord_sig = sig;
    const int64_t n = (int64_t)S->ncols, nnz = S->nvals;
    if (n + (int64_t)(1 << 22) > 0x7fffffff || nnz >= 0xf0000000ll) return;
    const size_t vb = S->type->size;
    const int64_t k_hot = hot_table_size(n, vb);
    if (k_hot < 64 || n < ctx().hot_min_cols) return;
    DevBuf<unsigned int> poscnt(n);
    const bool ranked = S->ranked;
    const int64_t m_rows = (int64_t)S->nrows;
    if (S->order.col_order_only && !S->order.perm) S->order.col_order_only = false;
    const bool col_only = !ranked && S->order.col_order_only;
    if (!ranked && !col_only && S->nrows != S->ncols) return;
    GB_Perm *P = ranked ? nullptr : (col_only ? S->order.perm : ensure_perm(S, k_hot, poscnt));
    GB_Matrix_opaque *R = matrix_new(S->type, S->nrows, S->ncols);
    try {
      if (col_only) {
        DevBuf<unsigned int> cnt(n, true);
        const int hstride = nnz >= ((int64_t)1 << 26) ? 8 : 1;
        hipLaunchKernelGGL(k_hot_hist, dim3((unsigned)ceil_div(nnz, 256 * hstride)), dim3(256), 0, ctx().stream, S->d_col, nnz, cnt.p, hstride);
        hipLaunchKernelGGL(k_order_poscnt, dim3((unsigned)ceil_div(n, 256)), dim3(256), 0, ctx().stream, (const unsigned int *)cnt.p,
                           (const int32_t *)P->d_inv, n, poscnt.p);
        R->d_ptr = (int64_t *)dev_alloc(sizeof(int64_t) * (size_t)(m_rows + 1));
        d2d(R->d_ptr, matrix_rowptr(S), sizeof(int64_t) * (size_t)(m_rows + 1));
// ... 275 lines not shown
    A->split.rtile = std::move(rt);
}

template <typename T, int MON, int MUL, int IPT>
static void launch_pull_ipt(GB_Matrix_opaque *A, PullArgs &a)
{
    using W = typename Widen<T>::type;
    const bool use_split = A->split.split_state == 1 && a.aval == A->d_val &&
                           a.col == (A->split.split_hot ? A->col_hot() : A->d_col) && a.n_chunks > 0;
    if (use_split) {
        GB_Matrix_opaque *S = A->split.short_part.get();
        DevBuf<W> tl_val((GRB_STRIP_ABL & 32) ? std::max<int64_t>(a.n_long, (A->split.strips.strip_cb[A->split.strips.strip_ncls > 0 ? A->split.strips.strip_ncls : 0] + 1) * 64) : a.n_long);
        DevBuf<unsigned char> tl_has(a.n_long);
        const bool by_strip = (A->split.split_kind == 2 || A->split.split_kind == 4) && A->split.long_nnz > 0 && (A->split.strips.strip_nseg > 0 || A->split.cold.ct_units > 0);
        ctx().stats.long_entries = A->nvals - S->nvals;
        ctx().stats.long_segments = by_strip ? A->split.strips.strip_nseg : 0;
        const bool by_class = A->split.split_kind == 1 && A->split.long_nnz > 0 && A->split.n_items > 0;
        ctx().stats.long_kernel = by_strip ? A->split.split_kind : (by_class ? 1 : 0);
        a.long_tails = A->split.tails_max_len > 0 ? 1 : 0;
        ctx().stats.long_tails = a.long_tails;
        DevBuf<uint32_t> long_act((size_t)ceil_div(a.n_long, 64) * 2);
        a.long_act = long_act.p;
        bool hot_fast = false;
        if constexpr (MON >= 0) hot_fast = hstrip_fast_semiring<T>(MON, MUL) && A->split.split_kind == 4 && by_strip && a.u_full && a.need_uval && a.need_aval && !a.a_iso;
        if (hot_fast) {
            const int rec_ct = A->vd.vdict_n > 0 ? 24 : 16 + 8 * (int)sizeof(T);
            int64_t widest = 0;
            for (int c = 0; c < A->split.strips.strip_ncls + A->split.strips.hub_ncls; c++) widest = std::max<int64_t>(widest, A->split.strips.strip_cb[c + 1] - A->split.strips.strip_cb[c]);
            if (A->split.strips.hrec_bytes != rec_ct || widest * 64 * (int64_t)A->split.strips.hrec_bytes >= (1ll << 31)) hot_fast = false;
        }
        DevBuf<unsigned char> long_act8(hot_fast && a.has_mask ? (size_t)a.n_long : 1);
        a.long_act8 = long_act8.p;
        LongProbe pb{nullptr, 0, nullptr, nullptr, nullptr, 0u};
        if constexpr (std::is_same<T, bool>::value && ((MON == OP_LOR && MUL == OP_LAND) || (MON == OP_ANY && MUL == OP_PAIR))) {
            if (by_class && A->split.d_probe && ctx().bool_probe > 0 && !a.u_full && (a.u_pv != nullptr || !a.need_uval) && (a.a_iso || !a.need_aval) &&
                a.col == (A->split.split_hot ? A->col_hot() : A->d_col)) {
                pb.probe = A->split.d_probe;
                pb.k = std::min(ctx().bool_probe, A->split.probe_k);
                pb.pv = a.u_pv;
                pb.pbits = a.u_pv ? nullptr : (const uint32_t *)a.u_bits;
                pb.iso_val = a.need_aval ? (const bool *)a.aval : nullptr;
                pb.want = MON == OP_LOR ? 2u : 1u;
                ctx().stats.long_probe = pb.k;
            }
        }
        hipLaunchKernelGGL((k_long_init<W>), dim3((unsigned)ceil_div(a.n_long, 256)), dim3(256), 0, ctx().stream, tl_val.p, tl_has.p,
                           a.n_long, pull_seed<T, W>(a, a.monoid), a.long_rows, a.m_bits, a.has_mask, a.m_comp, long_act.p,
                           ((by_class || by_strip) && a.u_full) ? 1 : 0, (by_strip && acc_is_ordered<W>(a.monoid)) ? 1 : 0,
                           (hot_fast && a.has_mask) ? long_act8.p : nullptr, A->split.rtile.rt_state == 1 ? A->split.rtile.d_rt_counter.get() : nullptr, pb);
        a.tl_ord = (by_strip && acc_is_ordered<W>(a.monoid)) ? 1 : 0;
        a.long_has_known = ((by_class || by_strip) && a.u_full) ? 1 : 0;
        a.tl_val = tl_val.p;
        a.tl_has = tl_has.p;
        a.dbg = ctx().debug_flags;
        const int64_t ncb = ceil_div(A->split.n_items, (int64_t)COMPACT_BLOCK);
        const bool compact = by_class && (a.has_mask || pb.probe != nullptr);
        DevBuf<int64_t> act_start(compact ? (size_t)A->split.n_items : 1), block_cnt(compact ? (size_t)ncb + 1 : 1), class_off(9);
        DevBuf<int32_t> act_len(compact ? (size_t)A->split.n_items : 1), act_slot(compact ? (size_t)A->split.n_items : 1);
        if (by_strip) {
            a.lcol = A->split.d_lcol;
            a.lval = A->split.d_lval;
            a.cls_lds_lim = A->split.cls_lds_lim;
            a.strip_start = A->split.strips.d_sstart;
            a.strip_slot = A->split.strips.d_sslot;
            a.strip_slot16 = A->split.strips.d_sslot16;
            a.strip_slot_base = A->split.strips.d_sslot_base;
            a.strip_nseg = A->split.strips.strip_nseg;
            for (int c = 0; c <= A->split.strips.strip_ncls; c++) a.strip_cb[c] = A->split.strips.strip_cb[c];
            a.strip_ncls = A->split.strips.strip_ncls;
            const int64_t G = std::max<int64_t>(A->split.strips.strip_ncls, (int64_t)(ctx().num_cus / A->split.strips.strip_ncls) * A->split.strips.strip_ncls);
            if (A->split.split_kind == 4) {
                a.hrec = A->split.strips.d_hrec;
                a.hrec_bytes = A->split.strips.hrec_bytes;
                a.vdict = A->vd.vdict_n > 0 ? A->vd.d_vdict.get() : nullptr;
                ctx().stats.value_dict = A->vd.vdict_n;
                auto launch_ctile = [&]() {
                    if (A->split.cold.ct_units <= 0) return;
                    a.ct_col = A->split.cold.d_ct_col;
                    a.ct_val = A->split.cold.d_ct_val;
                    a.ct_loc = A->split.cold.d_ct_loc;
                    a.ct_tiles = (const CTile *)A->split.cold.d_ct_tiles.get();
                    a.ct_mode = A->split.cold.ct_mode;
                    const int ctm = A->split.cold.ct_mode;
                    a.ct_cbase = (ctm == 1 || ctm == 2) ? (const int32_t *)((const char *)A->split.cold.d_ct_tiles.get() + sizeof(CTile) * (size_t)std::max<int64_t>(A->split.cold.ct_ntiles, 1)) : nullptr;
                    if (ctm == 2 || ctm == 3) a.vdict = A->vd.d_vdict;
                    ctx().stats.cold_tile_mode = ctm;
                    a.ct_order = A->split.cold.d_ct_order;
                    for (int x = 0; x <= 8; x++) a.ct_xoff[x] = A->split.cold.ct_xoff[x];
                    const int64_t Gt = std::max<int64_t>(8, (int64_t)(ctx().num_cus * CT_WGS_PER_CU / 8) * 8);
                    if (ctm == 3) {
                        if constexpr (sizeof(T) == 4 && !std::is_same<T, bool>::value)
                            hipLaunchKernelGGL((k_mxv_ctile<T, MON, MUL, true>), dim3((unsigned)Gt), dim3(CT_BLOCK), 0, ctx().stream, a);
                        else
                            fail(GrB_PANIC, "cold tiles: code words built for a type that has no kernel for them (internal error)");
                    } else
                    hipLaunchKernelGGL((k_mxv_ctile<T, MON, MUL>), dim3((unsigned)Gt), dim3(CT_BLOCK), 0, ctx().stream, a);
                    ctx().stats.kernel_launches += 1;
                };
                bool merged = false;
                if constexpr (MON >= 0) {
                    if constexpr (hstrip_fast_semiring<T>(MON, MUL)) {
                        if (hot_fast && A->split.strips.hub_ncls > 0 && A->split.strips.d_wg_tab && A->split.strips.wg_tab_g > 0 && A->split.strips.strip_cb[A->split.strips.strip_ncls + A->split.strips.hub_ncls] > 0) {
                            PullArgs al = a;
                            al.wg_tab = A->split.strips.d_wg_tab;
                            al.strip_cb_dev = A->split.strips.d_strip_cb;
                            al.strip_chunks = A->split.strips.strip_cb[A->split.strips.strip_ncls + A->split.strips.hub_ncls];
                            bool dict_launched = false;
                            const bool s16 = al.strip_slot16 != nullptr;
                            if constexpr (sizeof(T) == 4) {
                                if (al.vdict) {
                                    if (s16) hipLaunchKernelGGL((k_mxv_hstrip<T, MON, MUL, LONG_LDS_WORDS, true, true>), dim3((unsigned)A->split.strips.wg_tab_g), dim3(LONG_BLOCK), 0, ctx().stream, al);
                                    else hipLaunchKernelGGL((k_mxv_hstrip<T, MON, MUL, LONG_LDS_WORDS, true>), dim3((unsigned)A->split.strips.wg_tab_g), dim3(LONG_BLOCK), 0, ctx().stream, al);
                                    dict_launched = true;
                                }
                            }
                            if (!dict_launched) {
                                if (s16) hipLaunchKernelGGL((k_mxv_hstrip<T, MON, MUL, LONG_LDS_WORDS, false, true>), dim3((unsigned)A->split.strips.wg_tab_g), dim3(LONG_BLOCK), 0, ctx().stream, al);
                                else hipLaunchKernelGGL((k_mxv_hstrip<T, MON, MUL, LONG_LDS_WORDS>), dim3((unsigned)A->split.strips.wg_tab_g), dim3(LONG_BLOCK), 0, ctx().stream, al);
                            }
                            merged = true;
                        }
                    }
                }
                for (int level = 0; !merged && level < (A->split.strips.hub_ncls > 0 ? 2 : 1); level++) {
                    const int c0 = level ? A->split.strips.strip_ncls : 0, nc = level ? A->split.strips.hub_ncls : A->split.strips.strip_ncls;
                    if (A->split.strips.strip_cb[c0 + nc] == A->split.strips.strip_cb[c0]) continue;
                    PullArgs al = a;
                    al.strip_ncls = nc;
                    for (int c = 0; c <= nc; c++) al.strip_cb[c] = A->split.strips.strip_cb[c0 + c];
                    al.cls_lds_lim = level ? A->split.strips.hub_lds_lim : A->split.cls_lds_lim;
                    const int64_t Gl = std::max<int64_t>(nc, (int64_t)(ctx().num_cus / nc) * nc);
                    bool launched = false;
                    if constexpr (MON >= 0) {
                        if constexpr (hstrip_fast_semiring<T>(MON, MUL)) {
                            if (hot_fast) {
                                bool dict_launched = false;
                                const bool s16 = al.strip_slot16 != nullptr;
                                if constexpr (sizeof(T) == 4) {
                                    if (al.vdict) {
                                        if (s16) hipLaunchKernelGGL((k_mxv_hstrip<T, MON, MUL, LONG_LDS_WORDS, true, true>), dim3((unsigned)Gl), dim3(LONG_BLOCK), 0, ctx().stream, al);
                                        else hipLaunchKernelGGL((k_mxv_hstrip<T, MON, MUL, LONG_LDS_WORDS, true>), dim3((unsigned)Gl), dim3(LONG_BLOCK), 0, ctx().stream, al);
                                        dict_launched = true;
                                    }
                                }
                                if (!dict_launched) {
                                    if (s16) hipLaunchKernelGGL((k_mxv_hstrip<T, MON, MUL, LONG_LDS_WORDS, false, true>), dim3((unsigned)Gl), dim3(LONG_BLOCK), 0, ctx().stream, al);
                                    else hipLaunchKernelGGL((k_mxv_hstrip<T, MON, MUL, LONG_LDS_WORDS>), dim3((unsigned)Gl), dim3(LONG_BLOCK), 0, ctx().stream, al);
                                }
                                launched = true;
                            }
                        }
                    }
                    if (!launched)
                        hipLaunchKernelGGL((k_mxv_strip<T, MON, MUL, LONG_LDS_WORDS, 1>), dim3((unsigned)Gl), dim3(LONG_BLOCK), 0, ctx().stream, al);
                    if (level) ctx().stats.kernel_launches += 1;
                }
                launch_ctile();
            } else
            hipLaunchKernelGGL((k_mxv_strip<T, MON, MUL, LONG_LDS_WORDS>), dim3((unsigned)G), dim3(LONG_BLOCK), 0, ctx().stream, a);
        } else if (by_class) {
            a.lcol = A->split.d_lcol;
            a.lval = A->split.d_lval;
            a.it_start = A->split.d_it_start;
            a.it_len = A->split.d_it_len;
            a.it_slot = A->split.d_it_slot;
            for (int c = 0; c < 9; c++) a.item_begin[c] = A->split.item_begin[c];
            a.cls_lds_lim = A->split.cls_lds_lim;
            a.class_off = nullptr;
            if (compact) {
                hipLaunchKernelGGL(k_long_compact_count, dim3((unsigned)ncb), dim3(256), 0, ctx().stream, (const int32_t *)A->split.d_it_slot,
                                   A->split.n_items, (const uint32_t *)long_act.p, block_cnt.p);
                prim_exclusive_sum_i64(block_cnt.p, block_cnt.p, ncb + 1);
                hipLaunchKernelGGL(k_long_compact_write, dim3((unsigned)ncb), dim3(256), 0, ctx().stream, (const int32_t *)A->split.d_it_slot,
                                   A->split.n_items, (const uint32_t *)long_act.p, (const int64_t *)block_cnt.p,
                                   (const int64_t *)A->split.d_item_begin, (const int64_t *)A->split.d_it_start, (const int32_t *)A->split.d_it_len,
                                   act_start.p, act_len.p, act_slot.p, class_off.p);
                a.it_start = act_start.p;
// ... 865 lines not shown
            if (A->tr->order.ord) {
                matrix_free(A->tr->order.ord);
                A->tr->order.ord = nullptr;
            }
            A->tr->order.ord_state = 0;
            A->tr->ranked = A->ranked;
        }
    }
    GRB_CATCH(errp(A))
}

extern "C" GrB_Info GrX_Matrix_shard_setup(GrB_Matrix A, const uint32_t *col_counts, int on_device, const GrB_Matrix like)
{
    GRB_TRY
    require_init();
    check_matrix(A, "A");
    GB_Perm *P = nullptr;
    const int64_t n = (int64_t)A->ncols;
    if (like) {
        check_matrix(like, "like");
        if (!like->order.perm || !like->order.col_order_only || like->ncols != A->ncols) fail(GrB_INVALID_VALUE, "GrX_Matrix_shard_setup: `like` carries no column order of this width");
        P = like->order.perm;
        perm_retain(P);
    } else {
        if (!col_counts) fail(GrB_NULL_POINTER, "GrX_Matrix_shard_setup: col_counts is NULL");
        if (n <= 0 || n + (int64_t)(1 << 22) > 0x7fffffff) fail(GrB_NOT_IMPLEMENTED, "GrX_Matrix_shard_setup: column count out of range");
        DevBuf<unsigned int> cnt(n);
        if (on_device) d2d(cnt.p, col_counts, sizeof(unsigned int) * (size_t)n);
        else h2d(cnt.p, col_counts, sizeof(unsigned int) * (size_t)n);
        DevBuf<uint64_t> keys(n), keys2(n);
        DevBuf<uint32_t> ids(n), ids2(n);
        DevBuf<unsigned int> poscnt(n);
        hipLaunchKernelGGL(k_order_keys, dim3((unsigned)ceil_div(n, 256)), dim3(256), 0, ctx().stream, (const unsigned int *)cnt.p, (const int64_t *)nullptr, n, keys.p, ids.p);
        prim_sort_pairs_u64_u32(keys.p, keys2.p, ids.p, ids2.p, n, 40);
        P = new GB_Perm();
        P->n = (uint64_t)n;
        try {
            P->d_rank = (int32_t *)dev_alloc(sizeof(int32_t) * (size_t)n);
            P->d_inv = (int32_t *)dev_alloc(sizeof(int32_t) * (size_t)n);
            DevBuf<unsigned long long> live(2, true);
            const int64_t k_hot = hot_table_size(n, A->type->size);
            hipLaunchKernelGGL(k_order_place, dim3((unsigned)ceil_div(n, 1024)), dim3(1024), 0, ctx().stream, (const uint32_t *)ids2.p, (const uint64_t *)keys2.p, n, k_hot,
                               P->d_rank, P->d_inv, poscnt.p, live.p);
            unsigned long long h_live[2] = {0, 0};
            d2h(h_live, live.p, sizeof(h_live));
            P->n_live_rows = 0;
            P->n_live_cols = (int64_t)h_live[1];
        } catch (...) {
            perm_release(P);
            throw;
        }
        sync_stream();
    }
    if (A->order.ord) {
        matrix_free(A->order.ord);
        A->order.ord = nullptr;
    }
    A->order.ord_state = 0;
    perm_release(A->order.perm);
    A->order.perm = P;
    A->order.col_order_only = true;
    GRB_CATCH(errp(A))
}

uint64_t GB_Matrix_opaque::RowTiles::bytes(uint64_t vs, bool dict) const
{
    if (rt_state != 1) return 0;
    return (uint64_t)rt_units * RT_EPL * (6 + (d_rt_val ? (dict && vs == 4 ? 1 : vs) : 0)) + 36ull * (uint64_t)rt_ntiles;
}
uint64_t GB_Matrix_opaque::TaggedGroups::bytes(uint64_t nrows, uint64_t vs, bool dict) const
{
    if (tg_state == 1) return (uint64_t)tg_units * TAG_EPL * (5 + (d_tg_val ? (dict ? 1 : vs) : 0)) + 12ull * ((nrows + 63) / 64);
    if (tg_state == 2) return 12ull * ((nrows + 63) / 64);
    return 0;
}
uint64_t GB_Matrix_opaque::Strips::hot_bytes() const
{
    const uint64_t hot_lanes = (uint64_t)strip_cb[strip_ncls + hub_ncls] * 64;
    return hot_lanes * (uint64_t)hrec_bytes + (d_sslot16 ? hot_lanes * 2 + hot_lanes / 16 : hot_lanes * 4) + hot_lanes / 8;
}
uint64_t GB_Matrix_opaque::ColdTiles::bytes(uint64_t vs) const
{
    const uint64_t cold = (uint64_t)ct_units * CT_EPL;
    return cold * ((d_ct_loc ? 6 : 4) + (d_ct_val ? (ct_mode == 2 ? 1 : vs) : 0)) + 20ull * (uint64_t)ct_ntiles;
}
uint64_t GB_Matrix_opaque::RowSplit::bytes(uint64_t nrows, uint64_t vs, bool dict) const
{
    if (split_state != 1) return 0;
    const GB_Matrix_opaque *S = short_part.get();
    uint64_t b = 8ull * (nrows + 1) + (short_tagged_only ? 0 : 4ull * (uint64_t)S->nvals + (S->iso ? vs : vs * (uint64_t)S->nvals));
    b += bits_words64(nrows) * 8 + 4ull * (uint64_t)n_long + 4ull * bits_words64(nrows) + 16ull * (uint64_t)n_chunks;
    if (d_probe) b += 4ull * (uint64_t)probe_k * (uint64_t)n_long;
    b += rtile.bytes(vs, dict) + tagged.bytes(nrows, vs, dict);
    if (split_kind == 4 && (strips.strip_nseg > 0 || cold.ct_units > 0)) {
        b += strips.hot_bytes() + cold.bytes(vs);
    } else if (split_kind == 2 && strips.strip_nseg > 0) {
        const uint64_t padded = (uint64_t)strips.strip_cb[strips.strip_ncls] * STRIP_CH;
        b += padded * 4 + (d_lval ? padded * vs : 0) + padded / 2 + padded / STRIP_CH * 8;
    } else if (n_items > 0) {
        const uint64_t padded = (uint64_t)long_nnz + 4ull * (uint64_t)n_items;
        b += padded * 4 + (d_lval ? padded * vs : 0) + 16ull * (uint64_t)n_items;
    }
    return b;
}

extern "C" GrB_Info GrX_Matrix_cache_bytes(const GrB_Matrix A, uint64_t *bytes)
{
    GRB_TRY
    require_init();
    check_matrix(A, "A");
    if (!bytes) fail(GrB_NULL_POINTER, "bytes is NULL");
    uint64_t b = A->tile.bytes() + A->hot.bytes() + A->split.bytes(A->nrows, A->type->size, A->vd.vdict_n > 0);
    if (A->col_hot()) b += 4ull * (uint64_t)A->nvals;
    if (A->order.ord) {
        uint64_t tb = 0;
        (void)GrX_Matrix_cache_bytes(A->order.ord, &tb);
        b += tb + 8ull * (A->nrows + 1) + 8ull * A->nrows;
    }
    *bytes = b;
    GRB_CATCH(errp(A))
}

extern "C" GrB_Info GrB_Matrix_reduce_Monoid(GrB_Vector w, const GrB_Vector mask, const GrB_BinaryOp accum, const GrB_Monoid monoid,
                                             const GrB_Matrix A, const GrB_Descriptor desc)
{
    GRB_TRY
    require_init();
    check_vector_any(w, "w");
    if (mask) check_vector_any(mask, "mask");
    check_matrix(A, "A");
    if (!monoid) fail(GrB_NULL_POINTER, "monoid is NULL");
    DescFlags f = flags_of(desc);
    GB_Matrix_opaque *S = f.t0 ? matrix_transpose_cached(A) : A;
    f.t0 = false;
    const GB_Semiring_opaque sr = {monoid->op, OP_FIRST, monoid->type, "reduce"};
    GB_Vector_opaque *ones = vector_new(type_of_code(monoid->type), S->ncols);
    ones->d_val = dev_alloc(16);
    ones->d_bits = (uint64_t *)dev_alloc(16);
    ones->nvals = (int64_t)S->ncols;
    try {
        mxv_any_order(w, mask, accum, &sr, S, ones, false, f, true);
    } catch (...) {
        vector_free(ones);
        throw;
    }
    vector_free(ones);
    GRB_CATCH(errp(w))
}

namespace grb {
void preload_mxv() { hipFuncAttributes at; (void)hipFuncGetAttributes(&at, reinterpret_cast<const void *>(&k_hot_hist)); (void)hipGetLastError(); }
}
```

python-graphblas_amd/csrc/grb_mxv_common.inc:

```
constexpr int PULL_BLOCK = 256;

struct CTile;
struct RTile;
struct PullArgs {
    int64_t m, nnz;
    const int64_t *rowptr;
    const int32_t *col;
    const void *aval;
    int a_iso;
    const void *u_val;
    const uint32_t *u_bits;
    int u_full;
    int monoid, mult;
    int need_aval, need_uval;
    const int64_t *tile_row;
    int64_t n_tiles;
    const uint64_t *m_bits;
    int has_mask, m_comp;
    int accum, replace;
    const void *w_old_val;
    const uint64_t *w_old_bits;
    void *w_new_val;
    uint64_t *w_new_bits;
    int fresh;
    void *carry_val;
    uint8_t *carry_has;
    void *first_val;
    uint8_t *first_has;
    int stream_nt;
    const uint32_t *u_valbits;
    const uint32_t *u_pv;
    int64_t x_len;
    const uint64_t *long_bits;
    const int32_t *long_rows;
    const int32_t *chunk_slot;
    const int64_t *chunk_start;
    const int32_t *chunk_len;
    int64_t n_chunks, n_long;
    int64_t n_long_epi;
    const int32_t *long_prefix;
    const int32_t *lcol;
    const void *lval;
    const int64_t *it_start;
    const int32_t *it_len;
    const int32_t *it_slot;
    int64_t item_begin[9];
    int cls_lds_lim;
    const int64_t *class_off;
    int has_by_value;
    int long_has_known;
    uint32_t *long_act;
    unsigned char *long_act8;
    const unsigned long long *strip_start;
    const int32_t *strip_slot;
    const uint16_t *strip_slot16;
    const int32_t *strip_slot_base;
    int tl_ord;
    int64_t strip_nseg;
    int strip_ncls;
    int64_t strip_cb[65];
    const int32_t *ct_col;
    const void *ct_val;
    const uint16_t *ct_loc;
    const struct CTile *ct_tiles;
    int ct_mode;
    const int32_t *ct_cbase;
    const int32_t *ct_order;
    int64_t ct_xoff[9];
    const char *hrec;
    int hrec_bytes;
    const int32_t *wg_tab;
    const int64_t *strip_cb_dev;
    int64_t strip_chunks;
    const void *vdict;
    const int32_t *tg_off;
    const int32_t *tg_col;
    const void *tg_val;
    const unsigned char *tg_tag;
    const uint64_t *tg_nonempty;
    int64_t tg_groups;
    int64_t tg_stride;
    const int32_t *rt_col;
    const uint16_t *rt_tag;
    const void *rt_val;
    const struct RTile *rt_tiles;
    const int32_t *rt_order;
    unsigned int *rt_counter;
    int64_t rt_units;
    int rt_ntiles;
    int long_tails;
    void *tl_val;
    unsigned char *tl_has;
    long long *dbg_times;
    int dbg;
};

__global__ void k_tile_table(const int64_t *rowptr, int64_t m, int64_t nnz, int tile, int64_t n_tiles, int64_t *tile_row)
{
    const int64_t t = (int64_t)blockIdx.x * blockDim.x + threadIdx.x;
    if (t > n_tiles) return;
    const int64_t total = m + nnz;
    int64_t diag = t * (int64_t)tile;
    if (diag > total) diag = total;
    int64_t lo = diag - nnz > 0 ? diag - nnz : 0, hi = diag < m ? diag : m;
    while (lo < hi) {
        const int64_t mid = (lo + hi) >> 1;
        if (rowptr[mid + 1] <= diag - mid - 1) lo = mid + 1;
        else hi = mid;
    }
    tile_row[t] = lo;
}

template <typename T, typename W> GRB_HD W pull_seed(const PullArgs &a, int monoid)
{
    return a.has_by_value ? monoid_identity<T, W>(monoid) : acc_seed<T, W>(monoid);
}

template <typename T> __device__ __forceinline__ bool same_bits(T x, T y)
{
    if constexpr (sizeof(T) == 1) return __builtin_bit_cast(uint8_t, x) == __builtin_bit_cast(uint8_t, y);
    else if constexpr (sizeof(T) == 2) return __builtin_bit_cast(uint16_t, x) == __builtin_bit_cast(uint16_t, y);
    else if constexpr (sizeof(T) == 4) return __builtin_bit_cast(uint32_t, x) == __builtin_bit_cast(uint32_t, y);
    else return __builtin_bit_cast(uint64_t, x) == __builtin_bit_cast(uint64_t, y);
}
template <typename T>
__device__ __forceinline__ bool write_rule_row(const PullArgs &a, int64_t row, bool mact, bool old_has, T old_val, bool t_has,
                                               T t_val)
{
    T *w_new = (T *)a.w_new_val;
    if (!mact) {
        const bool keep = a.replace ? false : old_has;
        if (keep && a.fresh) w_new[row] = old_val;
        return keep;
    }
    if (a.accum >= 0) {
        if (old_has && t_has) {
            const T nv = apply_binop<T>(a.accum, old_val, t_val);
            if (a.fresh || !same_bits(nv, old_val)) w_new[row] = nv;
            return true;
        }
        if (old_has) { if (a.fresh) w_new[row] = old_val; return true; }
        if (t_has) { w_new[row] = t_val; return true; }
        return false;
    }
    if (t_has) w_new[row] = t_val;
    return t_has;
}

#if defined(__HIP_DEVICE_COMPILE__)
// ... 61 lines not shown
{
    const auto v = __builtin_amdgcn_raw_buffer_load_b128(r, byte_off, 0, 0);
    return make_uint4(v[0], v[1], v[2], v[3]);
}
typedef uint32_t grb_u32x4 __attribute__((ext_vector_type(4)));
typedef uint32_t grb_u32x2 __attribute__((ext_vector_type(2)));
__device__ __forceinline__ uint4 buf_stream_x4(__amdgpu_buffer_rsrc_t r, unsigned byte_off, bool nt)
{
    if (nt) {
        const auto v = __builtin_amdgcn_raw_buffer_load_b128(r, byte_off, 0, 2);
        return make_uint4(v[0], v[1], v[2], v[3]);
    }
    const auto v = __builtin_amdgcn_raw_buffer_load_b128(r, byte_off, 0, 0);
    return make_uint4(v[0], v[1], v[2], v[3]);
}
__device__ __forceinline__ uint2 buf_stream_x2(__amdgpu_buffer_rsrc_t r, unsigned byte_off, bool nt)
{
    if (nt) {
        const auto v = __builtin_amdgcn_raw_buffer_load_b64(r, byte_off, 0, 2);
        return make_uint2(v[0], v[1]);
    }
    const auto v = __builtin_amdgcn_raw_buffer_load_b64(r, byte_off, 0, 0);
    return make_uint2(v[0], v[1]);
}
__device__ __forceinline__ uint32_t buf_stream_x1(__amdgpu_buffer_rsrc_t r, unsigned byte_off, bool nt)
{
    if (nt) return (uint32_t)__builtin_amdgcn_raw_buffer_load_b32(r, byte_off, 0, 2);
    return (uint32_t)__builtin_amdgcn_raw_buffer_load_b32(r, byte_off, 0, 0);
}
__device__ __forceinline__ uint4 ptr_stream_x4(const void *p, bool nt)
{
#if defined(__HIP_DEVICE_COMPILE__)
    if (nt) {
        const grb_u32x4 v = __builtin_nontemporal_load((const grb_u32x4 *)p);
        return make_uint4(v[0], v[1], v[2], v[3]);
    }
#endif
    (void)nt;
    return *(const uint4 *)p;
}
__device__ __forceinline__ uint2 ptr_stream_x2(const void *p, bool nt)
{
#if defined(__HIP_DEVICE_COMPILE__)
    if (nt) {
        const grb_u32x2 v = __builtin_nontemporal_load((const grb_u32x2 *)p);
        return make_uint2(v[0], v[1]);
    }
#endif
    (void)nt;
    return *(const uint2 *)p;
}

constexpr int FILL_U = 13;
template <int BLOCK, typename E, typename F>
__device__ __forceinline__ void lds_fill(E *dst, int n, F load)
{
    for (int k0 = threadIdx.x; k0 < n; k0 += BLOCK * FILL_U) {
        E t[FILL_U];
#pragma unroll
        for (int u = 0; u < FILL_U; u++) {
            const int k = k0 + u * BLOCK;
            t[u] = E();
            if (k < n) t[u] = load(k);
        }
#pragma unroll
        for (int u = 0; u < FILL_U; u++) {
            const int k = k0 + u * BLOCK;
            if (k < n) dst[k] = t[u];
        }
    }
}

__device__ __forceinline__ int wave_inclusive_max_nonneg(int v)
{
    int t;
    t = __builtin_amdgcn_update_dpp(0, v, 0x111, 0xf, 0xf, false); v = v > t ? v : t;
    t = __builtin_amdgcn_update_dpp(0, v, 0x112, 0xf, 0xf, false); v = v > t ? v : t;
    t = __builtin_amdgcn_update_dpp(0, v, 0x114, 0xf, 0xf, false); v = v > t ? v : t;
    t = __builtin_amdgcn_update_dpp(0, v, 0x118, 0xf, 0xf, false); v = v > t ? v : t;
    t = __builtin_amdgcn_update_dpp(0, v, 0x142, 0xa, 0xf, false); v = v > t ? v : t;
    t = __builtin_amdgcn_update_dpp(0, v, 0x143, 0xc, 0xf, false); v = v > t ? v : t;
    return v;
}
__device__ __forceinline__ int wave_lane_below(int v, int first) { return __builtin_amdgcn_update_dpp(first, v, 0x138, 0xf, 0xf, false); }
```

python-graphblas_amd/csrc/grb_mxv_ctile.inc:

```
#ifndef GRB_CT_SLOTS
#define GRB_CT_SLOTS 16384
#endif
#ifndef GRB_CT_BLOCK
#define GRB_CT_BLOCK 1024
#endif
constexpr int CT_SLOTS = GRB_CT_SLOTS;
constexpr int CT_PACK_SLOTS = 8192, CT_PACK_COLBITS = 19;
constexpr int CT_BLOCK = GRB_CT_BLOCK;
constexpr int CT_EPL = 4;
#ifndef GRB_CT_WGS_PER_CU
#define GRB_CT_WGS_PER_CU 2
#endif
constexpr int CT_WGS_PER_CU = GRB_CT_WGS_PER_CU;
#ifndef GRB_CT_ABL
#define GRB_CT_ABL 0
#endif
struct alignas(16) CTile {
    int64_t u0;
    int32_t n_units;
    int32_t base;
};
template <typename W> struct CtSlots { static constexpr int value = sizeof(W) > 4 ? CT_SLOTS / 2 : CT_SLOTS; };

#ifndef GRB_CT_MAX_ENTRIES
#define GRB_CT_MAX_ENTRIES 16384
#endif
constexpr int64_t CT_MAX_ENTRIES = GRB_CT_MAX_ENTRIES;
__global__ void k_ctile_first(const uint64_t *skeys, int64_t n, int64_t n_tiles, int n_sb, unsigned v0, int64_t *first, int slots)
{
    const int64_t t = (int64_t)blockIdx.x * blockDim.x + threadIdx.x;
    if (t > n_tiles) return;
    const uint64_t want = (((uint64_t)v0 + (uint64_t)(t / n_sb)) << 32) | (uint64_t)((t % n_sb) * (int64_t)slots);
    int64_t lo = 0, hi = n;
    while (lo < hi) {
        const int64_t mid = (lo + hi) >> 1;
        if (skeys[mid] < want) lo = mid + 1;
        else hi = mid;
    }
    first[t] = lo;
}
__global__ void k_ctile_keys2(const uint32_t *sidx, int64_t p0, int64_t n_cold, const int64_t *efirst, int64_t n_tiles, const int32_t *col,
                              uint64_t *key2, uint32_t *pay)
{
    const int64_t c = (int64_t)blockIdx.x * blockDim.x + threadIdx.x;
    if (c >= n_cold) return;
    const int64_t p = p0 + c;
    int64_t lo = 0, hi = n_tiles;
    while (hi - lo > 1) {
        const int64_t mid = (lo + hi) >> 1;
        if (efirst[mid] <= p) lo = mid;
        else hi = mid;
    }
    key2[c] = ((uint64_t)lo << 32) | (uint64_t)(uint32_t)col[sidx[p]];
    pay[c] = (uint32_t)c;
}
template <typename T>
__global__ void k_ctile_place(const uint64_t *skeys, const uint32_t *sidx, int64_t p0, int64_t n_cold, const uint64_t *key2s, const uint32_t *pays,
                              const int64_t *efirst, const CTile *tiles, const T *val, int iso, int32_t *tcol, T *tval, uint16_t *tloc,
                              const unsigned long long *vd_table, const unsigned char *vd_codes, const int32_t *cbase, int code_word)
{
    const int64_t q = (int64_t)blockIdx.x * blockDim.x + threadIdx.x;
    if (q >= n_cold) return;
    const uint64_t k2 = key2s[q];
    const int64_t t = (int64_t)(k2 >> 32);
    const int64_t p = p0 + (int64_t)pays[q];
    const int64_t slot = (int64_t)(uint32_t)skeys[p];
    const int64_t d = tiles[t].u0 * CT_EPL + (q - (efirst[t] - p0));
    if (cbase) tcol[d] = (int32_t)((((uint32_t)(slot - tiles[t].base)) << CT_PACK_COLBITS) | (((uint32_t)k2 - (uint32_t)cbase[t]) & ((1u << CT_PACK_COLBITS) - 1u)));
    else tcol[d] = (int32_t)(uint32_t)k2;
    bool coded = false;
    if constexpr (sizeof(T) == 4) {
        if (vd_table) {
            const uint32_t code = (uint32_t)vdict_code(vd_table, vd_codes, ((const uint32_t *)val)[sidx[p]]) & 0xffu;
            if (code_word) tcol[d] = (int32_t)((code << 24) | ((uint32_t)k2 & 0x00ffffffu));
            else ((unsigned char *)tval)[d] = (unsigned char)code;
            coded = true;
        }
    }
    if (!iso && !coded) tval[d] = val[sidx[p]];
    if (tloc) tloc[d] = (uint16_t)(slot - tiles[t].base);
}

__global__ void k_ctile_pad_slots(const CTile *tiles, const int64_t *efirst, int64_t n_tiles, uint16_t *tloc, uint16_t pad_slot)
{
    const int64_t t = (int64_t)blockIdx.x * blockDim.x + threadIdx.x;
    if (t >= n_tiles) return;
    const int64_t d0 = tiles[t].u0 * CT_EPL, d1 = d0 + (int64_t)tiles[t].n_units * CT_EPL;
    for (int64_t d = d0 + (efirst[t + 1] - efirst[t]); d < d1; d++) tloc[d] = pad_slot;
}

template <typename T, int MONOID_CT, int MULT_CT, bool CODEW = false>
__global__ __launch_bounds__(CT_BLOCK) void k_mxv_ctile(const PullArgs a)
{
    using W = typename Widen<T>::type;
    constexpr int EPL = CT_EPL, SLOTS = CtSlots<W>::value;
    static_assert(!CODEW || (sizeof(T) == 4 && !std::is_same<T, bool>::value && SLOTS == CT_SLOTS), "code words: 4-byte values, tiles of CT_SLOTS slots");
    __shared__ W s_acc[SLOTS];
    __shared__ uint32_t s_off[SLOTS / 32 + (CODEW ? 1 : 0)];
    __shared__ uint32_t s_has[SLOTS / 32];
    __shared__ uint32_t s_dict[sizeof(T) == 4 ? 256 : 1];
    const int monoid = MONOID_CT >= 0 ? MONOID_CT : a.monoid;
    const int mult = MULT_CT >= 0 ? MULT_CT : a.mult;
    const bool need_aval = a.need_aval != 0, need_uval = a.need_uval != 0;
    const bool stage_vals = need_aval && !a.a_iso;
    const bool snt = a.stream_nt != 0;
    const T iso_v = (a.a_iso && need_aval) ? ((const T *)a.aval)[0] : (T)0;
    const __amdgpu_buffer_rsrc_t xval_rs = make_rsrc(a.u_val, a.x_len * (int64_t)sizeof(T));
    const __amdgpu_buffer_rsrc_t xbits_rs = make_rsrc(a.u_bits, a.u_full ? 0 : ((a.x_len + 63) >> 6) * 8);
    const __amdgpu_buffer_rsrc_t xvbits_rs = make_rsrc(a.u_valbits, a.u_valbits ? ((a.x_len + 63) >> 6) * 8 : 0);
    const __amdgpu_buffer_rsrc_t xpv_rs = make_rsrc(a.u_pv, a.u_pv ? ((a.x_len + 15) >> 4) * 4 : 0);
    const int32_t *tcol = a.ct_col;
    const T *tval = (const T *)a.ct_val;
    const uint16_t *tloc = a.ct_loc;
    W *tl = (W *)a.tl_val;
    const W ident = pull_seed<T, W>(a, monoid);
    const int packed = CODEW ? 0 : a.ct_mode;
    const int slots_rt = packed ? (CT_PACK_SLOTS < SLOTS ? CT_PACK_SLOTS : SLOTS) : SLOTS;
    if constexpr (CODEW) {
        for (int i = threadIdx.x; i < 256; i += CT_BLOCK) s_dict[i] = ((const uint32_t *)a.vdict)[i];
        if (threadIdx.x == 0) s_off[SLOTS / 32] = ~0u;
    } else if constexpr (sizeof(T) == 4) {
        if (packed == 2) {
            for (int i = threadIdx.x; i < 256; i += CT_BLOCK) s_dict[i] = ((const uint32_t *)a.vdict)[i];
            __syncthreads();
        }
    }
    const int xcd = (int)(blockIdx.x & 7u), li = (int)(blockIdx.x >> 3), nx = (int)(gridDim.x >> 3);
    const int64_t x0 = a.ct_xoff[xcd], x1 = a.ct_xoff[xcd + 1];
    for (int64_t tl_i = x0 + li; tl_i < x1; tl_i += nx) {
        const CTile tile = a.ct_tiles[a.ct_order[tl_i]];
        if (tile.n_units == 0) continue;
        const int cbase = packed ? a.ct_cbase[a.ct_order[tl_i]] : 0;
        const int rows_here = (int)((a.n_long - tile.base < slots_rt) ? a.n_long - tile.base : slots_rt);
        for (int i = threadIdx.x; i < slots_rt; i += CT_BLOCK) s_acc[i] = ident;
        for (int i = threadIdx.x; i < slots_rt / 32; i += CT_BLOCK) {
            s_has[i] = 0u;
            const int64_t wd = ((int64_t)tile.base >> 5) + i;
            s_off[i] = (a.has_mask && (int64_t)i * 32 < rows_here) ? ~a.long_act[wd] : 0u;
        }
        __syncthreads();
        const int64_t u_end = tile.u0 + tile.n_units;
        constexpr int UB = 1;
        for (int64_t ub0 = tile.u0; ub0 < u_end; ub0 += (int64_t)CT_BLOCK * UB) {
            const int64_t ub = ub0 + threadIdx.x;
            int creg[UB][EPL], rk[UB][EPL], cc[UB][EPL];
            T vreg[UB][EPL];
            unsigned vcode[UB][EPL];
            bool uv[UB];
#pragma unroll
            for (int k = 0; k < UB; k++) {
                const int64_t u = ub + (int64_t)k * CT_BLOCK;
                uv[k] = u < u_end;
                const int64_t e = (uv[k] ? u : u_end - 1) * EPL;
                const uint4 c4 = ptr_stream_x4(tcol + e, snt);
                creg[k][0] = (int)c4.x; creg[k][1] = (int)c4.y; creg[k][2] = (int)c4.z; creg[k][3] = (int)c4.w;
                if constexpr (CODEW) {
                    const uint2 l2 = ptr_stream_x2(tloc + e, snt);
                    rk[k][0] = (int)(l2.x & 0xffffu); rk[k][1] = (int)(l2.x >> 16); rk[k][2] = (int)(l2.y & 0xffffu); rk[k][3] = (int)(l2.y >> 16);
#pragma unroll
                    for (int i = 0; i < EPL; i++) {
                        const unsigned w = (unsigned)creg[k][i];
                        creg[k][i] = (int)(w & 0x00ffffffu);
                        vcode[k][i] = w >> 24;
                    }
                } else if (packed) {
#pragma unroll
                    for (int i = 0; i < EPL; i++) {
                        const unsigned w = (unsigned)creg[k][i];
                        rk[k][i] = (int)(w >> CT_PACK_COLBITS);
                        creg[k][i] = w == 0xffffffffu ? -1 : cbase + (int)(w & ((1u << CT_PACK_COLBITS) - 1u));
                        if (w == 0xffffffffu) rk[k][i] = 0;
                    }
                } else {
                    const uint2 l2 = ptr_stream_x2(tloc + e, snt);
                    rk[k][0] = (int)(l2.x & 0xffffu); rk[k][1] = (int)(l2.x >> 16); rk[k][2] = (int)(l2.y & 0xffffu); rk[k][3] = (int)(l2.y >> 16);
                }
                bool vals_done = CODEW;
                if constexpr (sizeof(T) == 4 && !CODEW) {
                    if (stage_vals && packed == 2) {
                        const uint32_t cd = ((const uint32_t *)tval)[uv[k] ? u : u_end - 1];
#pragma unroll
                        for (int i = 0; i < EPL; i++) vreg[k][i] = __builtin_bit_cast(T, s_dict[(cd >> (8 * i)) & 0xffu]);
                        vals_done = true;
                    }
                }
                if (vals_done) {
                } else if (stage_vals) {
                    if constexpr (sizeof(T) == 4) {
                        const uint4 v4 = ptr_stream_x4(tval + e, snt);
                        vreg[k][0] = __builtin_bit_cast(T, v4.x); vreg[k][1] = __builtin_bit_cast(T, v4.y);
                        vreg[k][2] = __builtin_bit_cast(T, v4.z); vreg[k][3] = __builtin_bit_cast(T, v4.w);
                    } else {
#pragma unroll
                        for (int i = 0; i < EPL; i++) vreg[k][i] = tval[e + i];
                    }
                } else {
#pragma unroll
                    for (int i = 0; i < EPL; i++) vreg[k][i] = iso_v;
                }
            }
#pragma unroll
            for (int k = 0; k < UB; k++)
#pragma unroll
                for (int i = 0; i < EPL; i++)
                    cc[k][i] = uv[k] ? (creg[k][i] | -(int)((s_off[rk[k][i] >> 5] >> (rk[k][i] & 31)) & 1u)) : -1;
            bool xp[UB][EPL];
            T xv[UB][EPL];
            bool pv_done = false;
            if constexpr (std::is_same<T, bool>::value) {
                if (a.u_pv) {
#pragma unroll
                    for (int k = 0; k < UB; k++) bool_pv_gather<EPL>(xpv_rs, cc[k], xp[k], xv[k]);
                    pv_done = true;
                }
            }
            if (pv_done) {
            } else if (a.u_full) {
#pragma unroll
                for (int k = 0; k < UB; k++)
#pragma unroll
                    for (int i = 0; i < EPL; i++) xp[k][i] = cc[k][i] >= 0;
            } else {
                uint32_t bw[UB][EPL];
#pragma unroll
                for (int k = 0; k < UB; k++)
#pragma unroll
                    for (int i = 0; i < EPL; i++) bw[k][i] = buf_load<uint32_t>(xbits_rs, (unsigned)(cc[k][i] >> 5) * 4u);
#pragma unroll
                for (int k = 0; k < UB; k++)
#pragma unroll
                    for (int i = 0; i < EPL; i++) xp[k][i] = (bw[k][i] >> (cc[k][i] & 31)) & 1u;
            }
            if (pv_done) {
            } else if (need_uval) {
                if constexpr (std::is_same<T, bool>::value) {
                    uint32_t vw[UB][EPL];
#pragma unroll
                    for (int k = 0; k < UB; k++)
#pragma unroll
                        for (int i = 0; i < EPL; i++) vw[k][i] = buf_load<uint32_t>(xvbits_rs, xp[k][i] ? (unsigned)(cc[k][i] >> 5) * 4u : 0xfffffff8u);
#pragma unroll
                    for (int k = 0; k < UB; k++)
#pragma unroll
                        for (int i = 0; i < EPL; i++) xv[k][i] = (vw[k][i] >> (cc[k][i] & 31)) & 1u;
                } else if (GRB_CT_ABL & 1) {
#pragma unroll
                    for (int k = 0; k < UB; k++)
#pragma unroll
                        for (int i = 0; i < EPL; i++) xv[k][i] = vreg[k][i];
                } else {
#pragma unroll
                    for (int k = 0; k < UB; k++)
#pragma unroll
                        for (int i = 0; i < EPL; i++) xv[k][i] = buf_gather<T>(xval_rs, xp[k][i] ? (unsigned)cc[k][i] * (unsigned)sizeof(T) : 0xfffffff8u);
                }
            } else {
#pragma unroll
                for (int k = 0; k < UB; k++)
#pragma unroll
                    for (int i = 0; i < EPL; i++) xv[k][i] = (T)0;
            }
            if constexpr (CODEW) {
#pragma unroll
                for (int k = 0; k < UB; k++)
#pragma unroll
                    for (int i = 0; i < EPL; i++) vreg[k][i] = stage_vals ? __builtin_bit_cast(T, s_dict[vcode[k][i]]) : iso_v;
            }
#pragma unroll
            for (int k = 0; k < UB; k++)
#pragma unroll
                for (int i = 0; i < EPL; i++) {
                    if (!xp[k][i]) continue;
                    const int r = rk[k][i];
                    const T prod = apply_binop<T>(mult, need_aval ? vreg[k][i] : (T)0, xv[k][i]);
                    if (GRB_CT_ABL & 4) { if (prod == (T)12345) s_acc[r] = (W)prod; atomicOr(&s_has[r >> 5], 1u << (r & 31)); continue; }
                    if (monoid == OP_ANY) s_acc[r] = (W)prod;
                    else lds_combine<W>(&s_acc[r], (W)prod, monoid);
                    atomicOr(&s_has[r >> 5], 1u << (r & 31));
                }
        }
        __syncthreads();
        if (GRB_CT_ABL & 2) continue;
        for (int i = threadIdx.x; i < rows_here; i += CT_BLOCK) {
            if (!((s_has[i >> 5] >> (i & 31)) & 1u)) continue;
            const int64_t s = tile.base + i;
            if (monoid == OP_ANY) tl[s] = s_acc[i];
            else if (a.tl_ord) atomic_combine_ord<W>(&tl[s], s_acc[i], monoid);
            else atomic_combine<W>(&tl[s], s_acc[i], monoid);
            if (!a.long_has_known) a.tl_has[s] = 1;
        }
        __syncthreads();
    }
}
```

Measured before the change: 289.4.

## Encode cold tiles as delta-coded gap words with packed slot and value code

Adds a new cold-tile layout (mode 4) in which each entry is a single 32-bit word holding a 10-bit column gap, the row slot and an 8-bit value-dictionary code. Per-block base columns are rebuilt in the kernel with a wave-wide prefix sum, and large gaps are written as escape words. This drops the separate 16-bit location stream and value stream, so the memory-bound mxv reads fewer bytes per nonzero. In exchange it adds escape and padding words, a wave scan per load, and extra sort and count work during layout construction. It is only chosen when escapes stay rare.

```diff
diff --git a/include/grb_mi355x.h b/include/grb_mi355x.h
--- a/include/grb_mi355x.h
+++ b/include/grb_mi355x.h
@@ -239,6 +239,8 @@
     int64_t long_tails;
     int64_t pinned_natural;
     int64_t cold_tile_mode;
+    int64_t cold_tile_escapes;
+    int64_t cold_tile_words;
 } GrX_Stats;
 GrB_Info GrX_last_stats(GrX_Stats *stats);
 GrB_Info GrX_mxm_streamed(const GrB_Semiring semiring, const GrB_Matrix A, const GrB_Matrix B, uint64_t budget_bytes,
diff --git a/python-graphblas_amd/_lib.py b/python-graphblas_amd/_lib.py
--- a/python-graphblas_amd/_lib.py
+++ b/python-graphblas_amd/_lib.py
@@ -24,7 +24,8 @@
                 ("out_nvals", ctypes.c_int64), ("method", ctypes.c_int32), ("fused_epilogue", ctypes.c_int32),
                 ("hot_k", ctypes.c_int64), ("long_entries", ctypes.c_int64), ("long_segments", ctypes.c_int64),
                 ("long_kernel", ctypes.c_int32), ("reorders", ctypes.c_int32), ("ordered", ctypes.c_int64), ("value_dict", ctypes.c_int64), ("fill_absent", ctypes.c_int64),
-                ("long_probe", ctypes.c_int64), ("long_tails", ctypes.c_int64), ("pinned_natural", ctypes.c_int64), ("cold_tile_mode", ctypes.c_int64)]
+                ("long_probe", ctypes.c_int64), ("long_tails", ctypes.c_int64), ("pinned_natural", ctypes.c_int64), ("cold_tile_mode", ctypes.c_int64),
+                ("cold_tile_escapes", ctypes.c_int64), ("cold_tile_words", ctypes.c_int64)]
 
 
 def load(path: str | None = None):
diff --git a/python-graphblas_amd/csrc/grb_context.hip b/python-graphblas_amd/csrc/grb_context.hip
--- a/python-graphblas_amd/csrc/grb_context.hip
+++ b/python-graphblas_amd/csrc/grb_context.hip
@@ -221,7 +221,8 @@
 bool short_kernel_exists(int64_t &v) { return v != 2 && v != 3 && v != 4; }
 bool snap_long_classes(int64_t &v) { if (v != 16 && v != 32 && v != 64) v = 8; return true; }
 bool window_group(int64_t &v) { return (v & (v - 1)) == 0; }
-bool explicit_cold_layout(int64_t &) { ctx().ctile_code = 0; return true; }
+bool explicit_cold_layout(int64_t &) { ctx().ctile_code = 0; ctx().ctile_gap = 0; return true; }
+bool explicit_code_layout(int64_t &) { ctx().ctile_gap = 0; return true; }
 bool release_cache_when_off(int64_t &v) { if (!v) dev_cache_release(); return true; }
 
 const Option OPTIONS[] = {
@@ -263,7 +264,8 @@
     opt("rows_tile", &Context::rows_tile, Option::WITHIN, 0, 2),
     opt("lazy_tagged", &Context::lazy_tagged, Option::WITHIN, 0, 1),
     opt("ctile_pack", &Context::ctile_pack, Option::WITHIN, 0, 2, explicit_cold_layout),
-    opt("ctile_code", &Context::ctile_code, Option::WITHIN, 0, 1),
+    opt("ctile_code", &Context::ctile_code, Option::WITHIN, 0, 1, explicit_code_layout),
+    opt("ctile_gap", &Context::ctile_gap, Option::WITHIN, 0, 1),
     opt("strip_slot16", &Context::strip_slot16, Option::WITHIN, 0, 1),
     opt("rtile_pack", &Context::rtile_pack, Option::WITHIN, 0, 1),
     opt("cold_in_rows", &Context::cold_in_rows, Option::CLAMP, 0, P30),
diff --git a/python-graphblas_amd/csrc/grb_internal.hpp b/python-graphblas_amd/csrc/grb_internal.hpp
--- a/python-graphblas_amd/csrc/grb_internal.hpp
+++ b/python-graphblas_amd/csrc/grb_internal.hpp
@@ -126,6 +126,7 @@
     int push_parity = 0;
     int lazy_tagged = 1;
     int ctile_code = 1;
+    int ctile_gap = 1;
     int ctile_pack = 0;
     int strip_slot16 = 1;
     int rtile_pack = 1;
@@ -334,6 +335,10 @@
         grb::DevPtr<void> d_ct_val;
         grb::DevPtr<uint16_t> d_ct_loc;
         grb::DevPtr<void> d_ct_tiles;
+        grb::DevPtr<int32_t> d_ct_gbase;
+        int64_t ct_gap_blocks = 0;
+        int64_t ct_escapes = 0;
+        int64_t ct_gap_words = 0;
         grb::DevPtr<int32_t> d_ct_order;
         int64_t ct_xoff[9] = {0};
         int64_t ct_ntiles = 0;
diff --git a/python-graphblas_amd/csrc/grb_mxv.hip b/python-graphblas_amd/csrc/grb_mxv.hip
--- a/python-graphblas_amd/csrc/grb_mxv.hip
+++ b/python-graphblas_amd/csrc/grb_mxv.hip
@@ -316,6 +316,7 @@
             std::vector<int32_t> h_bounds;
             if (kind == 4 && ctx().ctile_code == 1 && ctx().ctile_pack == 0 && A->vd.vdict_n > 0 && A->type->size == 4 && A->type->code != TC_BOOL && !A->iso && codes_total <= ((int64_t)1 << 24))
                 ct_mode = 3;
+            const bool gap_candidate = kind == 4 && ctx().ctile_gap == 1 && ctx().ctile_pack == 0 && A->vd.vdict_n > 0 && A->type->size == 4 && A->type->code != TC_BOOL && !A->iso;
             if (kind == 4 && own_ranges && ctx().ctile_pack > 0) {
                 h_bounds.resize((size_t)A->order.ct_ncr + 1);
                 d2h(h_bounds.data(), A->order.d_cold_bounds, sizeof(int32_t) * h_bounds.size());
@@ -492,7 +493,6 @@
                     sync_stream();
                 }
             }
-            const bool use_dict_all = ct_mode == 2 || ct_mode == 3;
             if (kind == 4 && nnz_long > n_strip) {
                 std::vector<CTile> h_tiles;
                 std::vector<int64_t> h_efirst;
@@ -542,9 +542,50 @@
                         if (range_xcd[(size_t)tile_range[(size_t)t]] == x) h_order.push_back((int32_t)t);
                 }
                 sp.cold.ct_xoff[8] = (int64_t)h_order.size();
+                DevBuf<int64_t> efirst(nt + 1);
+                h2d(efirst.p, h_efirst.data(), sizeof(int64_t) * (size_t)(nt + 1));
+                const int64_t n_cold = nnz_long - n_strip;
+                DevBuf<uint64_t> key2(n_cold), key2s(n_cold);
+                DevBuf<uint32_t> pay(n_cold), pays(n_cold);
+                hipLaunchKernelGGL(k_ctile_keys2, dim3((unsigned)ceil_div(n_cold, 256)), dim3(256), 0, ctx().stream, (const uint32_t *)idx2.p, n_strip, n_cold,
+                                   (const int64_t *)efirst.p, nt, col_src, key2.p, pay.p);
+                int tbits = 1;
+                while (((int64_t)1 << tbits) < nt) tbits++;
+                prim_sort_pairs_u64_u32(key2.p, key2s.p, pay.p, pays.p, n_cold, 32 + tbits);
+                DevBuf<int64_t> gwords(gap_candidate ? n_cold + 1 : 0), gtw(gap_candidate ? nt + 1 : 0);
+                sp.cold.ct_escapes = sp.cold.ct_gap_words = 0;
+                std::vector<int32_t> h_blk0;
+                int64_t gap_blocks = 0;
+                if (gap_candidate) {
+                    hipLaunchKernelGGL(k_ctile_gap_count, dim3((unsigned)ceil_div(n_cold + 1, 256)), dim3(256), 0, ctx().stream, (const uint64_t *)key2s.p, n_cold, gwords.p);
+                    prim_exclusive_sum_i64(gwords.p, gwords.p, n_cold + 1);
+                    hipLaunchKernelGGL(k_ctile_gap_tilewords, dim3((unsigned)ceil_div(nt + 1, 256)), dim3(256), 0, ctx().stream, (const int64_t *)gwords.p,
+                                       (const int64_t *)efirst.p, n_strip, nt, gtw.p);
+                    std::vector<int64_t> h_tw((size_t)nt + 1);
+                    d2h(h_tw.data(), gtw.p, sizeof(int64_t) * (size_t)(nt + 1));
+                    sp.cold.ct_gap_words = h_tw[(size_t)nt];
+                    sp.cold.ct_escapes = h_tw[(size_t)nt] - n_cold;
+                    if (sp.cold.ct_escapes * 20 <= sp.cold.ct_gap_words) {
+                        ct_mode = 4;
+                        units = 0;
+                        h_blk0.resize((size_t)nt);
+                        for (int big = 1; big >= 0; big--)
+                            for (int64_t t = 0; t < nt; t++) {
+                                const int64_t tw = h_tw[(size_t)t + 1] - h_tw[(size_t)t];
+                                if ((tw >= CT_GAP_ALIGN_MIN) != (big == 1)) continue;
+                                h_tiles[(size_t)t].u0 = units;
+                                h_tiles[(size_t)t].n_units = (int32_t)(big ? ceil_div(tw, (int64_t)CT_GAP_BLOCK) * (CT_GAP_BLOCK / CT_EPL) : ceil_div(tw, (int64_t)CT_EPL));
+                                units += h_tiles[(size_t)t].n_units;
+                                h_blk0[(size_t)t] = (int32_t)gap_blocks;
+                                gap_blocks += ceil_div(tw, (int64_t)CT_GAP_BLOCK);
+                            }
+                    }
+                }
+                const bool use_dict_all = ct_mode >= 2;
                 const size_t ents = (size_t)std::max<int64_t>(units, 1) * CT_EPL;
                 sp.cold.d_ct_tiles.reset(dev_alloc((sizeof(CTile) + sizeof(int32_t)) * (size_t)std::max<int64_t>(nt, 1)));
                 h2d(sp.cold.d_ct_tiles, h_tiles.data(), sizeof(CTile) * (size_t)nt);
+                if (ct_mode == 4) h2d((char *)sp.cold.d_ct_tiles.get() + sizeof(CTile) * (size_t)std::max<int64_t>(nt, 1), h_blk0.data(), sizeof(int32_t) * (size_t)nt);
                 if (ct_packed) {
                     std::vector<int32_t> h_cbase((size_t)nt);
                     for (int64_t t = 0; t < nt; t++) h_cbase[(size_t)t] = h_bounds[(size_t)tile_range[(size_t)t]];
@@ -552,9 +593,24 @@
                 }
                 sp.cold.d_ct_order.reset((int32_t *)dev_alloc(sizeof(int32_t) * (size_t)std::max<int64_t>(nt, 1)));
                 h2d(sp.cold.d_ct_order, h_order.data(), sizeof(int32_t) * (size_t)nt);
-                DevBuf<int64_t> efirst(nt + 1);
-                h2d(efirst.p, h_efirst.data(), sizeof(int64_t) * (size_t)(nt + 1));
                 sp.cold.d_ct_col.reset((int32_t *)dev_alloc(sizeof(int32_t) * ents));
+                if (ct_mode == 4) {
+                    sp.cold.d_ct_val.reset(nullptr);
+                    sp.cold.d_ct_loc.reset(nullptr);
+                    sp.cold.d_ct_gbase.reset((int32_t *)dev_alloc(sizeof(int32_t) * (size_t)std::max<int64_t>(gap_blocks, 1)));
+                    sp.cold.ct_gap_blocks = gap_blocks;
+                    hipLaunchKernelGGL(k_ctile_gap_pad, dim3((unsigned)ceil_div(nt, 256)), dim3(256), 0, ctx().stream, (const CTile *)sp.cold.d_ct_tiles.get(),
+                                       (const int64_t *)gtw.p, nt, sp.cold.d_ct_col.get());
+                    GRB_DISPATCH_TYPE(A->type->code, T, {
+                        hipLaunchKernelGGL((k_ctile_gap_place<T>), dim3((unsigned)ceil_div(n_cold, 256)), dim3(256), 0, ctx().stream, (const uint64_t *)keys2.p,
+                                           (const uint32_t *)idx2.p, n_strip, n_cold, (const uint64_t *)key2s.p, (const uint32_t *)pays.p, (const int64_t *)gwords.p,
+                                           (const int64_t *)gtw.p, (const CTile *)sp.cold.d_ct_tiles.get(),
+                                           (const int32_t *)((const char *)sp.cold.d_ct_tiles.get() + sizeof(CTile) * (size_t)std::max<int64_t>(nt, 1)), (const T *)A->d_val, sp.cold.d_ct_col.get(),
+                                           sp.cold.d_ct_gbase.get(), (const unsigned long long *)A->vd.d_vd_table, (const unsigned char *)A->vd.d_vd_codes);
+                    })
+                    sync_stream();
+                } else {
+                sp.cold.d_ct_gbase.reset(nullptr);
                 const size_t ct_vb = use_dict_all ? 1 : A->type->size;
                 sp.cold.d_ct_val.reset((A->iso || ct_mode == 3) ? nullptr : dev_alloc(ct_vb * ents));
                 sp.cold.d_ct_loc.reset(ct_packed ? nullptr : (uint16_t *)dev_alloc(sizeof(uint16_t) * ents));
@@ -564,25 +620,16 @@
                 if (ct_mode == 3 && nt > 0)
                     hipLaunchKernelGGL(k_ctile_pad_slots, dim3((unsigned)ceil_div(nt, 256)), dim3(256), 0, ctx().stream, (const CTile *)sp.cold.d_ct_tiles.get(),
                                        (const int64_t *)efirst.p, nt, sp.cold.d_ct_loc.get(), (uint16_t)ct_slots);
-                const int64_t n_cold = nnz_long - n_strip;
-                {
-                    DevBuf<uint64_t> key2(n_cold), key2s(n_cold);
-                    DevBuf<uint32_t> pay(n_cold), pays(n_cold);
-                    hipLaunchKernelGGL(k_ctile_keys2, dim3((unsigned)ceil_div(n_cold, 256)), dim3(256), 0, ctx().stream, (const uint32_t *)idx2.p, n_strip, n_cold,
-                                       (const int64_t *)efirst.p, nt, col_src, key2.p, pay.p);
-                    int tbits = 1;
-                    while (((int64_t)1 << tbits) < nt) tbits++;
-                    prim_sort_pairs_u64_u32(key2.p, key2s.p, pay.p, pays.p, n_cold, 32 + tbits);
-                    GRB_DISPATCH_TYPE(A->type->code, T, {
-                        hipLaunchKernelGGL((k_ctile_place<T>), dim3((unsigned)ceil_div(n_cold, 256)), dim3(256), 0, ctx().stream, (const uint64_t *)keys2.p,
-                                           (const uint32_t *)idx2.p, n_strip, n_cold, (const uint64_t *)key2s.p, (const uint32_t *)pays.p, (const int64_t *)efirst.p,
-                                           (const CTile *)sp.cold.d_ct_tiles.get(), (const T *)A->d_val, A->iso ? 1 : 0, sp.cold.d_ct_col, (T *)sp.cold.d_ct_val.get(), sp.cold.d_ct_loc,
-                                           use_dict_all ? (const unsigned long long *)A->vd.d_vd_table : (const unsigned long long *)nullptr,
-                                           use_dict_all ? (const unsigned char *)A->vd.d_vd_codes : (const unsigned char *)nullptr,
-                                           ct_packed ? (const int32_t *)((const char *)sp.cold.d_ct_tiles.get() + sizeof(CTile) * (size_t)std::max<int64_t>(nt, 1)) : (const int32_t *)nullptr,
-                                           ct_mode == 3 ? 1 : 0);
-                    })
-                    sync_stream();
+                GRB_DISPATCH_TYPE(A->type->code, T, {
+                    hipLaunchKernelGGL((k_ctile_place<T>), dim3((unsigned)ceil_div(n_cold, 256)), dim3(256), 0, ctx().stream, (const uint64_t *)keys2.p,
+                                       (const uint32_t *)idx2.p, n_strip, n_cold, (const uint64_t *)key2s.p, (const uint32_t *)pays.p, (const int64_t *)efirst.p,
+                                       (const CTile *)sp.cold.d_ct_tiles.get(), (const T *)A->d_val, A->iso ? 1 : 0, sp.cold.d_ct_col, (T *)sp.cold.d_ct_val.get(), sp.cold.d_ct_loc,
+                                       use_dict_all ? (const unsigned long long *)A->vd.d_vd_table : (const unsigned long long *)nullptr,
+                                       use_dict_all ? (const unsigned char *)A->vd.d_vd_codes : (const unsigned char *)nullptr,
+                                       ct_packed ? (const int32_t *)((const char *)sp.cold.d_ct_tiles.get() + sizeof(CTile) * (size_t)std::max<int64_t>(nt, 1)) : (const int32_t *)nullptr,
+                                       ct_mode == 3 ? 1 : 0);
+                })
+                sync_stream();
                 }
                 sp.cold.ct_mode = ct_mode;
                 sp.cold.ct_ntiles = nt;
@@ -678,7 +725,7 @@
     const Context &c = ctx();
     uint64_t h = 1469598103934665603ull;
     const int64_t v[] = {c.long_kernel, c.short_kernel, c.long_classes, c.split_min_len, c.long_sub, c.long_sub_min_len, c.lean_min_nnz,
-                         c.split_min_nnz, c.hot_k, c.drop_hot_cols, c.hub_min_len, c.value_dict, c.rows_tile, c.rtile_rows, c.rtile_entries, c.cold_in_rows, c.rtile_pack, c.strip_slot16, c.ctile_pack, c.ctile_code, c.lazy_tagged};
+                         c.split_min_nnz, c.hot_k, c.drop_hot_cols, c.hub_min_len, c.value_dict, c.rows_tile, c.rtile_rows, c.rtile_entries, c.cold_in_rows, c.rtile_pack, c.strip_slot16, c.ctile_pack, c.ctile_code, c.ctile_gap, c.lazy_tagged};
     for (int64_t x : v) h = (h ^ (uint64_t)x) * 1099511628211ull;
     return h;
 }
@@ -1120,9 +1167,12 @@
                     a.ct_tiles = (const CTile *)A->split.cold.d_ct_tiles.get();
                     a.ct_mode = A->split.cold.ct_mode;
                     const int ctm = A->split.cold.ct_mode;
-                    a.ct_cbase = (ctm == 1 || ctm == 2) ? (const int32_t *)((const char *)A->split.cold.d_ct_tiles.get() + sizeof(CTile) * (size_t)std::max<int64_t>(A->split.cold.ct_ntiles, 1)) : nullptr;
-                    if (ctm == 2 || ctm == 3) a.vdict = A->vd.d_vdict;
+                    a.ct_cbase = (ctm == 1 || ctm == 2 || ctm == 4) ? (const int32_t *)((const char *)A->split.cold.d_ct_tiles.get() + sizeof(CTile) * (size_t)std::max<int64_t>(A->split.cold.ct_ntiles, 1)) : nullptr;
+                    if (ctm >= 2) a.vdict = A->vd.d_vdict;
+                    a.ct_gbase = A->split.cold.d_ct_gbase;
                     ctx().stats.cold_tile_mode = ctm;
+                    ctx().stats.cold_tile_escapes = A->split.cold.ct_escapes;
+                    ctx().stats.cold_tile_words = A->split.cold.ct_gap_words;
                     a.ct_order = A->split.cold.d_ct_order;
                     for (int x = 0; x <= 8; x++) a.ct_xoff[x] = A->split.cold.ct_xoff[x];
                     const int64_t Gt = std::max<int64_t>(8, (int64_t)(ctx().num_cus * CT_WGS_PER_CU / 8) * 8);
@@ -1131,6 +1181,11 @@
                             hipLaunchKernelGGL((k_mxv_ctile<T, MON, MUL, true>), dim3((unsigned)Gt), dim3(CT_BLOCK), 0, ctx().stream, a);
                         else
                             fail(GrB_PANIC, "cold tiles: code words built for a type that has no kernel for them (internal error)");
+                    } else if (ctm == 4) {
+                        if constexpr (sizeof(T) == 4 && !std::is_same<T, bool>::value)
+                            hipLaunchKernelGGL((k_mxv_ctile<T, MON, MUL, false, true>), dim3((unsigned)Gt), dim3(CT_BLOCK), 0, ctx().stream, a);
+                        else
+                            fail(GrB_PANIC, "cold tiles: gap words built for a type that has no kernel for them (internal error)");
                     } else
                     hipLaunchKernelGGL((k_mxv_ctile<T, MON, MUL>), dim3((unsigned)Gt), dim3(CT_BLOCK), 0, ctx().stream, a);
                     ctx().stats.kernel_launches += 1;
@@ -2162,7 +2217,7 @@
 uint64_t GB_Matrix_opaque::ColdTiles::bytes(uint64_t vs) const
 {
     const uint64_t cold = (uint64_t)ct_units * CT_EPL;
-    return cold * ((d_ct_loc ? 6 : 4) + (d_ct_val ? (ct_mode == 2 ? 1 : vs) : 0)) + 20ull * (uint64_t)ct_ntiles;
+    return cold * ((d_ct_loc ? 6 : 4) + (d_ct_val ? (ct_mode == 2 ? 1 : vs) : 0)) + 20ull * (uint64_t)ct_ntiles + (d_ct_gbase ? 4ull * (uint64_t)ct_gap_blocks : 0);
 }
 uint64_t GB_Matrix_opaque::RowSplit::bytes(uint64_t nrows, uint64_t vs, bool dict) const
 {
diff --git a/python-graphblas_amd/csrc/grb_mxv_common.inc b/python-graphblas_amd/csrc/grb_mxv_common.inc
--- a/python-graphblas_amd/csrc/grb_mxv_common.inc
+++ b/python-graphblas_amd/csrc/grb_mxv_common.inc
@@ -65,6 +65,7 @@
     const struct CTile *ct_tiles;
     int ct_mode;
     const int32_t *ct_cbase;
+    const int32_t *ct_gbase;
     const int32_t *ct_order;
     int64_t ct_xoff[9];
     const char *hrec;
@@ -292,4 +293,14 @@
     t = __builtin_amdgcn_update_dpp(0, v, 0x143, 0xc, 0xf, false); v = v > t ? v : t;
     return v;
 }
+__device__ __forceinline__ int wave_inclusive_add(int v)
+{
+    v += __builtin_amdgcn_update_dpp(0, v, 0x111, 0xf, 0xf, false);
+    v += __builtin_amdgcn_update_dpp(0, v, 0x112, 0xf, 0xf, false);
+    v += __builtin_amdgcn_update_dpp(0, v, 0x114, 0xf, 0xf, false);
+    v += __builtin_amdgcn_update_dpp(0, v, 0x118, 0xf, 0xf, false);
+    v += __builtin_amdgcn_update_dpp(0, v, 0x142, 0xa, 0xf, false);
+    v += __builtin_amdgcn_update_dpp(0, v, 0x143, 0xc, 0xf, false);
+    return v;
+}
 __device__ __forceinline__ int wave_lane_below(int v, int first) { return __builtin_amdgcn_update_dpp(first, v, 0x138, 0xf, 0xf, false); }
diff --git a/python-graphblas_amd/csrc/grb_mxv_ctile.inc b/python-graphblas_amd/csrc/grb_mxv_ctile.inc
--- a/python-graphblas_amd/csrc/grb_mxv_ctile.inc
+++ b/python-graphblas_amd/csrc/grb_mxv_ctile.inc
@@ -89,11 +89,63 @@
     for (int64_t d = d0 + (efirst[t + 1] - efirst[t]); d < d1; d++) tloc[d] = pad_slot;
 }
 
-template <typename T, int MONOID_CT, int MULT_CT, bool CODEW = false>
+constexpr int CT_GAP_BITS = 10, CT_GAP_ESC = (1 << CT_GAP_BITS) - 1, CT_GAP_BLOCK = 64 * CT_EPL;
+constexpr int64_t CT_GAP_ALIGN_MIN = 2048;
+static_assert(CT_SLOTS <= (1 << (24 - CT_GAP_BITS)), "gap words: the slot field holds a tile's slots");
+__global__ void k_ctile_gap_count(const uint64_t *key2s, int64_t n_cold, int64_t *words)
+{
+    const int64_t q = (int64_t)blockIdx.x * blockDim.x + threadIdx.x;
+    if (q > n_cold) return;
+    if (q == n_cold) { words[q] = 0; return; }
+    const uint64_t k2 = key2s[q], k1 = q > 0 ? key2s[q - 1] : ~k2;
+    const uint32_t gap = (k1 >> 32) == (k2 >> 32) ? (uint32_t)k2 - (uint32_t)k1 : 0u;
+    words[q] = 1 + (int64_t)(gap / (uint32_t)CT_GAP_ESC);
+}
+__global__ void k_ctile_gap_tilewords(const int64_t *wsum, const int64_t *efirst, int64_t p0, int64_t n_tiles, int64_t *tw)
+{
+    const int64_t t = (int64_t)blockIdx.x * blockDim.x + threadIdx.x;
+    if (t <= n_tiles) tw[t] = wsum[efirst[t] - p0];
+}
+__global__ void k_ctile_gap_pad(const CTile *tiles, const int64_t *tw, int64_t n_tiles, int32_t *tcol)
+{
+    const int64_t t = (int64_t)blockIdx.x * blockDim.x + threadIdx.x;
+    if (t >= n_tiles) return;
+    const int64_t d0 = tiles[t].u0 * CT_EPL, d1 = d0 + (int64_t)tiles[t].n_units * CT_EPL;
+    for (int64_t d = d0 + (tw[t + 1] - tw[t]); d < d1; d++) tcol[d] = CT_GAP_ESC;
+}
+template <typename T>
+__global__ void k_ctile_gap_place(const uint64_t *skeys, const uint32_t *sidx, int64_t p0, int64_t n_cold, const uint64_t *key2s, const uint32_t *pays,
+                                  const int64_t *wsum, const int64_t *tw, const CTile *tiles, const int32_t *blk0, const T *val, int32_t *tcol, int32_t *gbase,
+                                  const unsigned long long *vd_table, const unsigned char *vd_codes)
+{
+    const int64_t q = (int64_t)blockIdx.x * blockDim.x + threadIdx.x;
+    if (q >= n_cold) return;
+    if constexpr (sizeof(T) == 4) {
+        const uint64_t k2 = key2s[q], k1 = q > 0 ? key2s[q - 1] : ~k2;
+        const int64_t t = (int64_t)(k2 >> 32);
+        const uint32_t c = (uint32_t)k2;
+        const uint32_t before = (k1 >> 32) == (k2 >> 32) ? (uint32_t)k1 : c;
+        const uint32_t n_esc = (c - before) / (uint32_t)CT_GAP_ESC, gap = (c - before) % (uint32_t)CT_GAP_ESC;
+        const int64_t p = p0 + (int64_t)pays[q];
+        const uint32_t slot = (uint32_t)((int64_t)(uint32_t)skeys[p] - tiles[t].base);
+        const uint32_t code = (uint32_t)vdict_code(vd_table, vd_codes, ((const uint32_t *)val)[sidx[p]]) & 0xffu;
+        int32_t *tc = tcol + tiles[t].u0 * CT_EPL, *gb = gbase + blk0[t];
+        int64_t d = wsum[q] - tw[t];
+        for (uint32_t j = 0; j < n_esc; j++, d++) {
+            tc[d] = CT_GAP_ESC;
+            if ((d & (CT_GAP_BLOCK - 1)) == 0) gb[d / CT_GAP_BLOCK] = (int32_t)(before + j * (uint32_t)CT_GAP_ESC);
+        }
+        tc[d] = (int32_t)((code << 24) | (slot << CT_GAP_BITS) | gap);
+        if ((d & (CT_GAP_BLOCK - 1)) == 0) gb[d / CT_GAP_BLOCK] = (int32_t)(c - gap);
+    }
+}
+
+template <typename T, int MONOID_CT, int MULT_CT, bool CODEW = false, bool GAPW = false>
 __global__ __launch_bounds__(CT_BLOCK) void k_mxv_ctile(const PullArgs a)
 {
     using W = typename Widen<T>::type;
     constexpr int EPL = CT_EPL, SLOTS = CtSlots<W>::value;
+    static_assert(!(CODEW && GAPW) && (!GAPW || (sizeof(T) == 4 && !std::is_same<T, bool>::value && SLOTS == CT_SLOTS)), "gap words: 4-byte values, tiles of CT_SLOTS slots");
     static_assert(!CODEW || (sizeof(T) == 4 && !std::is_same<T, bool>::value && SLOTS == CT_SLOTS), "code words: 4-byte values, tiles of CT_SLOTS slots");
     __shared__ W s_acc[SLOTS];
     __shared__ uint32_t s_off[SLOTS / 32 + (CODEW ? 1 : 0)];
@@ -114,11 +166,11 @@
     const uint16_t *tloc = a.ct_loc;
     W *tl = (W *)a.tl_val;
     const W ident = pull_seed<T, W>(a, monoid);
-    const int packed = CODEW ? 0 : a.ct_mode;
+    const int packed = (CODEW || GAPW) ? 0 : a.ct_mode;
     const int slots_rt = packed ? (CT_PACK_SLOTS < SLOTS ? CT_PACK_SLOTS : SLOTS) : SLOTS;
-    if constexpr (CODEW) {
+    if constexpr (CODEW || GAPW) {
         for (int i = threadIdx.x; i < 256; i += CT_BLOCK) s_dict[i] = ((const uint32_t *)a.vdict)[i];
-        if (threadIdx.x == 0) s_off[SLOTS / 32] = ~0u;
+        if (CODEW && threadIdx.x == 0) s_off[SLOTS / 32] = ~0u;
     } else if constexpr (sizeof(T) == 4) {
         if (packed == 2) {
             for (int i = threadIdx.x; i < 256; i += CT_BLOCK) s_dict[i] = ((const uint32_t *)a.vdict)[i];
@@ -130,7 +182,7 @@
     for (int64_t tl_i = x0 + li; tl_i < x1; tl_i += nx) {
         const CTile tile = a.ct_tiles[a.ct_order[tl_i]];
         if (tile.n_units == 0) continue;
-        const int cbase = packed ? a.ct_cbase[a.ct_order[tl_i]] : 0;
+        const int cbase = (packed || GAPW) ? a.ct_cbase[a.ct_order[tl_i]] : 0;
         const int rows_here = (int)((a.n_long - tile.base < slots_rt) ? a.n_long - tile.base : slots_rt);
         for (int i = threadIdx.x; i < slots_rt; i += CT_BLOCK) s_acc[i] = ident;
         for (int i = threadIdx.x; i < slots_rt / 32; i += CT_BLOCK) {
@@ -146,6 +198,7 @@
             int creg[UB][EPL], rk[UB][EPL], cc[UB][EPL];
             T vreg[UB][EPL];
             unsigned vcode[UB][EPL];
+            bool esc[UB][EPL];
             bool uv[UB];
 #pragma unroll
             for (int k = 0; k < UB; k++) {
@@ -154,7 +207,24 @@
                 const int64_t e = (uv[k] ? u : u_end - 1) * EPL;
                 const uint4 c4 = ptr_stream_x4(tcol + e, snt);
                 creg[k][0] = (int)c4.x; creg[k][1] = (int)c4.y; creg[k][2] = (int)c4.z; creg[k][3] = (int)c4.w;
-                if constexpr (CODEW) {
+                if constexpr (GAPW) {
+                    const int64_t ulast = u_end - 1 - tile.u0, urel = ub0 - tile.u0 + (int64_t)k * CT_BLOCK + (threadIdx.x & ~63u);
+                    const int gb = a.ct_gbase[__builtin_amdgcn_readfirstlane(cbase + (int)((urel < ulast ? urel : ulast) >> 6))];
+                    int run = 0;
+#pragma unroll
+                    for (int i = 0; i < EPL; i++) {
+                        const unsigned w = (unsigned)creg[k][i];
+                        const int g = (int)(w & (unsigned)CT_GAP_ESC);
+                        run += g;
+                        esc[k][i] = g == CT_GAP_ESC;
+                        rk[k][i] = (int)((w >> CT_GAP_BITS) & (unsigned)(CT_SLOTS - 1));
+                        vcode[k][i] = w >> 24;
+                        creg[k][i] = run;
+                    }
+                    const int front = gb + wave_inclusive_add(run) - run;
+#pragma unroll
+                    for (int i = 0; i < EPL; i++) creg[k][i] += front;
+                } else if constexpr (CODEW) {
                     const uint2 l2 = ptr_stream_x2(tloc + e, snt);
                     rk[k][0] = (int)(l2.x & 0xffffu); rk[k][1] = (int)(l2.x >> 16); rk[k][2] = (int)(l2.y & 0xffffu); rk[k][3] = (int)(l2.y >> 16);
 #pragma unroll
@@ -175,8 +245,8 @@
                     const uint2 l2 = ptr_stream_x2(tloc + e, snt);
                     rk[k][0] = (int)(l2.x & 0xffffu); rk[k][1] = (int)(l2.x >> 16); rk[k][2] = (int)(l2.y & 0xffffu); rk[k][3] = (int)(l2.y >> 16);
                 }
-                bool vals_done = CODEW;
-                if constexpr (sizeof(T) == 4 && !CODEW) {
+                bool vals_done = CODEW || GAPW;
+                if constexpr (sizeof(T) == 4 && !CODEW && !GAPW) {
                     if (stage_vals && packed == 2) {
                         const uint32_t cd = ((const uint32_t *)tval)[uv[k] ? u : u_end - 1];
 #pragma unroll
@@ -203,7 +273,7 @@
             for (int k = 0; k < UB; k++)
 #pragma unroll
                 for (int i = 0; i < EPL; i++)
-                    cc[k][i] = uv[k] ? (creg[k][i] | -(int)((s_off[rk[k][i] >> 5] >> (rk[k][i] & 31)) & 1u)) : -1;
+                    cc[k][i] = (uv[k] && !(GAPW && esc[k][i])) ? (creg[k][i] | -(int)((s_off[rk[k][i] >> 5] >> (rk[k][i] & 31)) & 1u)) : -1;
             bool xp[UB][EPL];
             T xv[UB][EPL];
             bool pv_done = false;
@@ -260,7 +330,7 @@
 #pragma unroll
                     for (int i = 0; i < EPL; i++) xv[k][i] = (T)0;
             }
-            if constexpr (CODEW) {
+            if constexpr (CODEW || GAPW) {
 #pragma unroll
                 for (int k = 0; k < UB; k++)
 #pragma unroll
```

Result: slower. 285.3 (-1.4%).
